# duj12/ASR-2Pass

Hardware: AMD Instinct MI355X
Metric: audio-sec/sec (xRT) Paraformer-large offline, 30s utts (higher is better)
Workload: dtype f32 (operands staged as 2 fp16 planes = 22-23 significant bits, 3 products per block on the FP16 matrix cores, fp32 accumulate; error vs fp64 = the fp32 MFMA chain's)

## Files before the change

### asr-2pass_amd/csrc/gemm_p3.hip

```cpp
#include "kernels.h"
#include "launch_common.h"
#include "split_common.h"

#include <algorithm>
#include <atomic>

namespace pfhip {
namespace {

using f32x16 = __attribute__((ext_vector_type(16))) float;

constexpr int kPM = 128, kPN = 128, kPK = 16;
constexpr int kPRowB = 32;
constexpr int kPPlane = 128 * kPRowB;
constexpr int kPStage = 4 * kPPlane;
constexpr int kPRing = 4;
constexpr int kPCs = kPN + 4;
constexpr int kPLds = kPM * kPCs * 4 + kPM * 8;
static_assert(kPRing * kPStage <= kPLds, "the ring must fit");

__device__ __forceinline__ size_t image_off(int kstep, int row, int piece, int rows) {
  return ((size_t)kstep * rows + row) * kPRowB + (size_t)((piece ^ ((row >> 3) & 1)) << 4);
}

// ... 203 lines not shown
#define PFHIP_S3(kt) PFHIP_STEP(ga_, gb_, fa, fb, 3, 0, kclamp((kt) + 7))
  int kt = 0;
  for (; kt + 3 < nk; kt += 4) { PFHIP_S0(kt) PFHIP_S1(kt) PFHIP_S2(kt) PFHIP_S3(kt) }
  if (kt < nk) PFHIP_S0(kt)
  if (kt + 1 < nk) PFHIP_S1(kt)
  if (kt + 2 < nk) PFHIP_S2(kt)
#undef PFHIP_S0
#undef PFHIP_S1
#undef PFHIP_S2
#undef PFHIP_S3
#undef PFHIP_STEP
#undef PFHIP_D1
#undef PFHIP_M
#undef PFHIP_RA
#undef PFHIP_RB
#undef PFHIP_DMA
#undef PFHIP_DMA1
#undef PFHIP_SB
  PFHIP_STAMP
  asm volatile("s_waitcnt vmcnt(0)" ::: "memory");
  __syncthreads();
  PFHIP_STAMP
#ifndef PFHIP_P3_EPI
#define PFHIP_P3_EPI 0
#endif
  if (PFHIP_P3_EPI == 2) {
    if (M < 0) C[tid] = acc00[0] + acc01[1] + acc10[2] + acc11[3];
    return;
  }
#ifndef PFHIP_P3_STAMPS
  const bool do_store = PFHIP_P3_EPI != 1 || M < 0;
#endif

  float* const Cs = reinterpret_cast<float*>(lds);
  {
    float* cw = Cs + (wr * 64 + 4 * h) * kPCs + wc * 64 + r;
#pragma unroll
    for (int e = 0; e < 16; ++e) {
      const int ro = ((e & 3) + 8 * (e >> 2)) * kPCs;
      cw[ro] = acc00[e];
      cw[ro + 32] = acc01[e];
      cw[ro + 32 * kPCs] = acc10[e];
      cw[ro + 32 * kPCs + 32] = acc11[e];
    }
  }
  float2* const s_mr = reinterpret_cast<float2*>(lds + kPM * kPCs * 4);
  if (LN && tid < kPM) s_mr[tid] = ln_mr;
  __syncthreads();
  PFHIP_STAMP
#ifdef PFHIP_P3_STAMPS
  const bool do_store = !stamp_wg;
#define PFHIP_P3_STAMP_END if (stamping) { asm volatile("s_waitcnt vmcnt(0)" ::: "memory"); *dbg_at(n_stamp) = __builtin_amdgcn_s_memtime(); *dbg_at(n_stamp + 1) = __builtin_amdgcn_s_memrealtime(); }
#else
#define PFHIP_P3_STAMP_END
#endif

  if (kv_tile) {
    row_planes_tile<LN, kPM, kPThreads>(Cs, s_mr, m0, n0, M, N, inv_scale, bias, ln_colsum, Ph, Pl, rows_p, split_col, tid, do_store);
  } else if (OUT & 1) {
    const int c4 = e_c4, rsub = e_rsub, gcol = e_gcol;
    float4 cv[16];
    float2 mrv[16];
#pragma unroll
    for (int pass = 0; pass < 16; ++pass) {
      const int row = pass * 8 + rsub;
      cv[pass] = *reinterpret_cast<const float4*>(Cs + row * kPCs + 4 * c4);
      mrv[pass] = LN ? s_mr[row] : make_float2(0.f, 1.f);
    }
#ifdef PFHIP_P3_STAMPS
    { float keep = cv[15].x + mrv[15].x; asm volatile("" : "+v"(keep)); }
    PFHIP_STAMP
#endif
#pragma unroll
    for (int pass = 0; pass < 16; ++pass) {
      const int row = pass * 8 + rsub, grow = m0 + row;
      float4 v = cv[pass];
      v.x *= inv_scale; v.y *= inv_scale; v.z *= inv_scale; v.w *= inv_scale;
      if (LN) {
        const float2 mr = mrv[pass];
        v.x = mr.y * (v.x - mr.x * e_cs.x); v.y = mr.y * (v.y - mr.x * e_cs.y); v.z = mr.y * (v.z - mr.x * e_cs.z); v.w = mr.y * (v.w - mr.x * e_cs.w);
      }
      v.x += e_bv.x + e_r1[pass].x; v.y += e_bv.y + e_r1[pass].y; v.z += e_bv.z + e_r1[pass].z; v.w += e_bv.w + e_r1[pass].w;
      if (relu) { v.x = fmaxf(v.x, 0.f); v.y = fmaxf(v.y, 0.f); v.z = fmaxf(v.z, 0.f); v.w = fmaxf(v.w, 0.f); }
      if (do_store && grow < M && e_cols) *reinterpret_cast<float4*>(C + (size_t)grow * ldc + gcol) = v;
      if (OUT & 2) *reinterpret_cast<float4*>(Cs + row * kPCs + 4 * c4) = v;
      if (stats_out) tile_row_stats(v, grow, M, tn, tiles_n, c4, stats_out);
    }
#ifdef PFHIP_P3_STAMPS
    PFHIP_STAMP
#endif
    if (OUT & 2) __syncthreads();
  }
  if (OUT & 2) {
    const int row = tid & 127, grow = m0 + row;
    const float2 mr = (LN && OUT == 2) ? s_mr[row] : make_float2(0.f, 1.f);
#pragma unroll
    for (int jj = 0; jj < 4; ++jj) {
      const int j = (tid >> 7) + 2 * jj;
      float v[16];
#pragma unroll
      for (int c = 0; c < 4; ++c) {
        const float4 t = *reinterpret_cast<const float4*>(Cs + row * kPCs + 16 * j + 4 * c);
        v[4 * c] = t.x; v[4 * c + 1] = t.y; v[4 * c + 2] = t.z; v[4 * c + 3] = t.w;
      }
      if (OUT == 2) {
        const int gc = n0 + 16 * j;
#pragma unroll
        for (int c = 0; c < 4; ++c) {
          const float4 b4 = bias ? *reinterpret_cast<const float4*>(bias + gc + 4 * c) : make_float4(0.f, 0.f, 0.f, 0.f);
          const float4 s4 = LN ? *reinterpret_cast<const float4*>(ln_colsum + gc + 4 * c) : make_float4(0.f, 0.f, 0.f, 0.f);
          const float bb[4] = {b4.x, b4.y, b4.z, b4.w}, ss[4] = {s4.x, s4.y, s4.z, s4.w};
#pragma unroll
          for (int e = 0; e < 4; ++e) {
            float x = v[4 * c + e] * inv_scale;
            if (LN) x = mr.y * (x - mr.x * ss[e]);
            x += bb[e];
            if (relu) x = fmaxf(x, 0.f);
            v[4 * c + e] = x;
          }
        }
      }
      const int ksp = (n0 >> 4) + j;
#pragma unroll
      for (int pc = 0; pc < 2; ++pc) {
        const float w8[8] = {v[8 * pc], v[8 * pc + 1], v[8 * pc + 2], v[8 * pc + 3], v[8 * pc + 4], v[8 * pc + 5], v[8 * pc + 6], v[8 * pc + 7]};
        uint4 hh, ll;
        split8(w8, hh, ll);
        const size_t off = image_off(ksp, grow, pc, rows_p);
        if (do_store) {
          *reinterpret_cast<uint4*>(Ph + off) = hh;
          *reinterpret_cast<uint4*>(Pl + off) = ll;
        } else if (hh.x == 0x12345678u && ll.y == 0x9abcdef0u) {
          Ph[0] = 1;
        }
      }
    }
  }
  PFHIP_P3_STAMP_END
}
#undef PFHIP_P3_STAMP_END
#undef PFHIP_STAMP

constexpr int kQM = 256;
constexpr int kQThreads = 512;
constexpr int kQAPlane = kQM * kPRowB;
constexpr int kQWOff = 2 * kQAPlane;
constexpr int kQStage = kQWOff + 2 * kPPlane;
constexpr int kQLds = kPRing * kQStage;
static_assert(kPM * kPCs * 4 + kQM * 8 <= kQLds, "half of the C tile and the row statistics must fit the ring");
template <bool LN, int OUT>
__global__ __launch_bounds__(kQThreads, 2) void gemm_p3_256_kernel(
    const unsigned char* __restrict__ Ah, const unsigned char* __restrict__ Al, int rows_a, const unsigned char* __restrict__ Wh,
    const unsigned char* __restrict__ Wl, int rows_w, float* C, int ldc, unsigned char* __restrict__ Ph, unsigned char* __restrict__ Pl,
    int rows_p, const float* __restrict__ bias, const float* R1, int ldr1, int M, int N, int K, int tiles_n, int n_tiles, int gw, int relu,
    const float* __restrict__ ln_stats, int ln_tiles, float ln_eps, const float* __restrict__ ln_colsum, float* __restrict__ stats_out,
    float inv_scale, int* range_flag, int split_col) {
  extern __shared__ __attribute__((aligned(16))) unsigned char lds[];

  int tm, tn;
  tile_of_block(blockIdx.x, n_tiles, tiles_n, gw, tm, tn);
  const int m0 = tm * kQM, n0 = tn * kPN;
  const int tid = threadIdx.x, lane = tid & 63, wave = tid >> 6;
  const int wr = wave >> 1, wc = wave & 1;
  const int r = lane & 31, h = lane >> 5;

  const size_t ka = (size_t)rows_a * kPRowB, kw = (size_t)rows_w * kPRowB;
  const int arow = min(m0 + 32 * wave, rows_a - 32);
// ... 40 lines not shown
    PFHIP_QDMA1(gww + (size_t)(kdma) * kw, (wst) * kQStage + lds_w) PFHIP_SB;                                         \
    PFHIP_M(acc01, FA[0][0], FB[0][1])                                                                                \
    PFHIP_M(acc10, FA[0][1], FB[0][0])                                                                                \
    PFHIP_M(acc11, FA[0][1], FB[0][1])                                                                                \
    asm volatile("s_waitcnt vmcnt(6) lgkmcnt(0)\n\ts_barrier" ::: "memory");                                          \
    PFHIP_SB;                                                                                                         \
  }

  const int nk = K / kPK;
  auto kclamp = [&](int t) { return t < nk ? t : nk - 1; };
  PFHIP_QDMA(0, 0)
  PFHIP_QDMA(1, kclamp(1))
  PFHIP_QDMA(2, kclamp(2))
  PFHIP_QDMA(3, kclamp(3))
  asm volatile("s_waitcnt vmcnt(6)\n\ts_barrier" ::: "memory");
  PFHIP_RA(fa, 0, 0, 0) PFHIP_RA(fa, 0, 0, 1) PFHIP_RA(fa, 0, 1, 0) PFHIP_RA(fa, 0, 1, 1)
  PFHIP_RB(fb, 0, 0, 0) PFHIP_RB(fb, 0, 0, 1) PFHIP_RB(fb, 0, 1, 0) PFHIP_RB(fb, 0, 1, 1)
  asm volatile("s_waitcnt lgkmcnt(0)\n\ts_barrier" ::: "memory");
#define PFHIP_S0(kt) PFHIP_STEP(fa, fb, ga_, gb_, 0, 1, kclamp((kt) + 4))
#define PFHIP_S1(kt) PFHIP_STEP(ga_, gb_, fa, fb, 1, 2, kclamp((kt) + 5))
#define PFHIP_S2(kt) PFHIP_STEP(fa, fb, ga_, gb_, 2, 3, kclamp((kt) + 6))
#define PFHIP_S3(kt) PFHIP_STEP(ga_, gb_, fa, fb, 3, 0, kclamp((kt) + 7))
  int kt = 0;
  for (; kt + 3 < nk; kt += 4) { PFHIP_S0(kt) PFHIP_S1(kt) PFHIP_S2(kt) PFHIP_S3(kt) }
  if (kt < nk) PFHIP_S0(kt)
  if (kt + 1 < nk) PFHIP_S1(kt)
  if (kt + 2 < nk) PFHIP_S2(kt)
#undef PFHIP_S0
#undef PFHIP_S1
#undef PFHIP_S2
#undef PFHIP_S3
#undef PFHIP_STEP
#undef PFHIP_M
#undef PFHIP_RA
#undef PFHIP_RB
#undef PFHIP_QDMA
#undef PFHIP_QDMA1
#undef PFHIP_SB
  asm volatile("s_waitcnt vmcnt(0)" ::: "memory");
  __syncthreads();

  float* const Cs = reinterpret_cast<float*>(lds);
  float2* const s_mr = reinterpret_cast<float2*>(lds + kPM * kPCs * 4);
  if (LN && tid < kQM) s_mr[tid] = ln_mr;
#pragma unroll 1
  for (int hf = 0; hf < 2; ++hf) {
    if ((wr >> 1) == hf) {
      float* cw = Cs + ((wr & 1) * 64 + 4 * h) * kPCs + wc * 64 + r;
#pragma unroll
      for (int e = 0; e < 16; ++e) {
        const int ro = ((e & 3) + 8 * (e >> 2)) * kPCs;
        cw[ro] = acc00[e];
        cw[ro + 32] = acc01[e];
        cw[ro + 32 * kPCs] = acc10[e];
        cw[ro + 32 * kPCs + 32] = acc11[e];
      }
    }
    __syncthreads();
    const int mh = m0 + 128 * hf;
    if (OUT & 1) {
      const int c4 = tid & 31, rsub = tid >> 5;
      const int gcol = n0 + 4 * c4;
      float4 bv = make_float4(0.f, 0.f, 0.f, 0.f), cs4 = bv;
      if (bias && gcol + 3 < N) bv = *reinterpret_cast<const float4*>(bias + gcol);
      if (LN && gcol + 3 < N) cs4 = *reinterpret_cast<const float4*>(ln_colsum + gcol);
      float4 r1v[8];
#pragma unroll
      for (int pass = 0; pass < 8; ++pass) {
        const int grow = mh + pass * 16 + rsub;
        r1v[pass] = (R1 && grow < M && gcol + 3 < N) ? *reinterpret_cast<const float4*>(R1 + (size_t)grow * ldr1 + gcol)
                                                     : make_float4(0.f, 0.f, 0.f, 0.f);
      }
#pragma unroll
      for (int pass = 0; pass < 8; ++pass) {
        const int row = pass * 16 + rsub, grow = mh + row;
        float4 v = *reinterpret_cast<const float4*>(Cs + row * kPCs + 4 * c4);
        v.x *= inv_scale; v.y *= inv_scale; v.z *= inv_scale; v.w *= inv_scale;
        if (LN) {
          const float2 mr = s_mr[128 * hf + row];
          v.x = mr.y * (v.x - mr.x * cs4.x); v.y = mr.y * (v.y - mr.x * cs4.y); v.z = mr.y * (v.z - mr.x * cs4.z); v.w = mr.y * (v.w - mr.x * cs4.w);
        }
        v.x += bv.x + r1v[pass].x; v.y += bv.y + r1v[pass].y; v.z += bv.z + r1v[pass].z; v.w += bv.w + r1v[pass].w;
        if (relu) { v.x = fmaxf(v.x, 0.f); v.y = fmaxf(v.y, 0.f); v.z = fmaxf(v.z, 0.f); v.w = fmaxf(v.w, 0.f); }
        if (grow < M && gcol + 3 < N) *reinterpret_cast<float4*>(C + (size_t)grow * ldc + gcol) = v;
        if (OUT & 2) *reinterpret_cast<float4*>(Cs + row * kPCs + 4 * c4) = v;
        if (stats_out) tile_row_stats(v, grow, M, tn, tiles_n, c4, stats_out);
      }
      if (OUT & 2) __syncthreads();
    }
    if (OUT & 2) {
      const int row = tid & 127, grow = mh + row;
      const float2 mr = (LN && OUT == 2) ? s_mr[128 * hf + row] : make_float2(0.f, 1.f);
#pragma unroll
      for (int jj = 0; jj < 2; ++jj) {
        const int j = (tid >> 7) + 4 * jj;
        float v[16];
#pragma unroll
        for (int c = 0; c < 4; ++c) {
          const float4 t = *reinterpret_cast<const float4*>(Cs + row * kPCs + 16 * j + 4 * c);
          v[4 * c] = t.x; v[4 * c + 1] = t.y; v[4 * c + 2] = t.z; v[4 * c + 3] = t.w;
        }
        if (OUT == 2) {
          const int gc = n0 + 16 * j;
#pragma unroll
          for (int c = 0; c < 4; ++c) {
            const float4 b4 = bias ? *reinterpret_cast<const float4*>(bias + gc + 4 * c) : make_float4(0.f, 0.f, 0.f, 0.f);
            const float4 s4 = LN ? *reinterpret_cast<const float4*>(ln_colsum + gc + 4 * c) : make_float4(0.f, 0.f, 0.f, 0.f);
            const float bb[4] = {b4.x, b4.y, b4.z, b4.w}, ss[4] = {s4.x, s4.y, s4.z, s4.w};
#pragma unroll
            for (int e = 0; e < 4; ++e) {
              float x = v[4 * c + e] * inv_scale;
              if (LN) x = mr.y * (x - mr.x * ss[e]);
              x += bb[e];
              if (relu) x = fmaxf(x, 0.f);
              v[4 * c + e] = x;
            }
          }
        }
        const int ksp = (n0 >> 4) + j;
        if (grow < rows_p) {
#pragma unroll
          for (int pc = 0; pc < 2; ++pc) {
            const float w8[8] = {v[8 * pc], v[8 * pc + 1], v[8 * pc + 2], v[8 * pc + 3], v[8 * pc + 4], v[8 * pc + 5], v[8 * pc + 6], v[8 * pc + 7]};
            uint4 hh, ll;
            split8(w8, hh, ll);
            const size_t off = image_off(ksp, grow, pc, rows_p);
            *reinterpret_cast<uint4*>(Ph + off) = hh;
            *reinterpret_cast<uint4*>(Pl + off) = ll;
          }
        }
      }
    }
    __syncthreads();
  }
}

template <bool LN, int OUT>
__device__ __forceinline__ void epilogue_rows64(const int tid, float* const Cs, const float2* const s_mr, const int m0, const int n0, const int tn,
                                                const int tiles_n, float* C, int ldc, unsigned char* __restrict__ Ph, unsigned char* __restrict__ Pl,
                                                int rows_p, const float* __restrict__ bias, const float* R1, int ldr1, int M, int N, int relu,
                                                const float* __restrict__ ln_colsum, float* __restrict__ stats_out, float inv_scale, int split_col) {
  if ((OUT & 4) && n0 >= split_col) {
    row_planes_tile<LN, 64, kPThreads>(Cs, s_mr, m0, n0, M, N, inv_scale, bias, ln_colsum, Ph, Pl, rows_p, split_col, tid, true);
  } else if (OUT & 1) {
    const int c4 = tid & 31, rsub = tid >> 5;
    const int gcol = n0 + 4 * c4;
    float4 bv = make_float4(0.f, 0.f, 0.f, 0.f), cs4 = bv;
    if (bias && gcol + 3 < N) bv = *reinterpret_cast<const float4*>(bias + gcol);
    if (LN && gcol + 3 < N) cs4 = *reinterpret_cast<const float4*>(ln_colsum + gcol);
    float4 r1v[8];
#pragma unroll
    for (int pass = 0; pass < 8; ++pass) {
      const int grow = m0 + pass * 8 + rsub;
      r1v[pass] = (R1 && grow < M && gcol + 3 < N) ? *reinterpret_cast<const float4*>(R1 + (size_t)grow * ldr1 + gcol)
                                                   : make_float4(0.f, 0.f, 0.f, 0.f);
    }
#pragma unroll
    for (int pass = 0; pass < 8; ++pass) {
      const int row = pass * 8 + rsub, grow = m0 + row;
      float4 v = *reinterpret_cast<const float4*>(Cs + row * kPCs + 4 * c4);
      v.x *= inv_scale; v.y *= inv_scale; v.z *= inv_scale; v.w *= inv_scale;
      if (LN) {
        const float2 mr = s_mr[row];
        v.x = mr.y * (v.x - mr.x * cs4.x); v.y = mr.y * (v.y - mr.x * cs4.y); v.z = mr.y * (v.z - mr.x * cs4.z); v.w = mr.y * (v.w - mr.x * cs4.w);
      }
      v.x += bv.x + r1v[pass].x; v.y += bv.y + r1v[pass].y; v.z += bv.z + r1v[pass].z; v.w += bv.w + r1v[pass].w;
      if (relu) { v.x = fmaxf(v.x, 0.f); v.y = fmaxf(v.y, 0.f); v.z = fmaxf(v.z, 0.f); v.w = fmaxf(v.w, 0.f); }
      if (grow < M && gcol + 3 < N) *reinterpret_cast<float4*>(C + (size_t)grow * ldc + gcol) = v;
      if (OUT & 2) *reinterpret_cast<float4*>(Cs + row * kPCs + 4 * c4) = v;
      if (stats_out) tile_row_stats(v, grow, M, tn, tiles_n, c4, stats_out);
    }
    if (OUT & 2) __syncthreads();
  }
  if (OUT & 2) {
    const int row = tid & 63, grow = m0 + row;
    const float2 mr = (LN && OUT == 2) ? s_mr[row] : make_float2(0.f, 1.f);
#pragma unroll
    for (int jj = 0; jj < 2; ++jj) {
      const int j = (tid >> 6) + 4 * jj;
      float v[16];
#pragma unroll
      for (int c = 0; c < 4; ++c) {
        const float4 t = *reinterpret_cast<const float4*>(Cs + row * kPCs + 16 * j + 4 * c);
        v[4 * c] = t.x; v[4 * c + 1] = t.y; v[4 * c + 2] = t.z; v[4 * c + 3] = t.w;
      }
      if (OUT == 2) {
        const int gc = n0 + 16 * j;
#pragma unroll
        for (int c = 0; c < 4; ++c) {
          const float4 b4 = bias ? *reinterpret_cast<const float4*>(bias + gc + 4 * c) : make_float4(0.f, 0.f, 0.f, 0.f);
          const float4 s4 = LN ? *reinterpret_cast<const float4*>(ln_colsum + gc + 4 * c) : make_float4(0.f, 0.f, 0.f, 0.f);
          const float bb[4] = {b4.x, b4.y, b4.z, b4.w}, ss[4] = {s4.x, s4.y, s4.z, s4.w};
#pragma unroll
          for (int e = 0; e < 4; ++e) {
            float x = v[4 * c + e] * inv_scale;
            if (LN) x = mr.y * (x - mr.x * ss[e]);
            x += bb[e];
            if (relu) x = fmaxf(x, 0.f);
            v[4 * c + e] = x;
          }
        }
      }
      const int ksp = (n0 >> 4) + j;
#pragma unroll
      for (int pc = 0; pc < 2; ++pc) {
        const float w8[8] = {v[8 * pc], v[8 * pc + 1], v[8 * pc + 2], v[8 * pc + 3], v[8 * pc + 4], v[8 * pc + 5], v[8 * pc + 6], v[8 * pc + 7]};
        uint4 hh, ll;
        split8(w8, hh, ll);
        const size_t off = image_off(ksp, grow, pc, rows_p);
        *reinterpret_cast<uint4*>(Ph + off) = hh;
        *reinterpret_cast<uint4*>(Pl + off) = ll;
      }
    }
  }
}

constexpr int kHM = 64;
constexpr int kHAPlane = kHM * kPRowB;
constexpr int kHWOff = 2 * kHAPlane;
constexpr int kHStage = kHWOff + 2 * kPPlane;
constexpr int kHLds = kPRing * kHStage;
static_assert(kHM * kPCs * 4 + kHM * 8 <= kHLds, "the C tile must fit the ring");
template <bool LN, int OUT>
__global__ __launch_bounds__(kPThreads, 3) void gemm_p3_64_kernel(
    const unsigned char* __restrict__ Ah, const unsigned char* __restrict__ Al, int rows_a, const unsigned char* __restrict__ Wh,
    const unsigned char* __restrict__ Wl, int rows_w, float* C, int ldc, unsigned char* __restrict__ Ph, unsigned char* __restrict__ Pl,
    int rows_p, const float* __restrict__ bias, const float* R1, int ldr1, int M, int N, int K, int tiles_n, int n_tiles, int gw, int relu,
    const float* __restrict__ ln_stats, int ln_tiles, float ln_eps, const float* __restrict__ ln_colsum, float* __restrict__ stats_out,
    float inv_scale, int* range_flag, int split_col) {
  extern __shared__ __attribute__((aligned(16))) unsigned char lds[];

  int tm, tn;
  tile_of_block(blockIdx.x, n_tiles, tiles_n, gw, tm, tn);
  const int m0 = tm * kHM, n0 = tn * kPN;
  const int tid = threadIdx.x, lane = tid & 63, wave = tid >> 6;
  const int wr = wave >> 1, wc = wave & 1;
  const int r = lane & 31, h = lane >> 5;

  const size_t ka = (size_t)rows_a * kPRowB, kw = (size_t)rows_w * kPRowB;
  const unsigned char* const ga = ((wave >> 1) ? Al : Ah) + ((size_t)(m0 + 32 * (wave & 1))) * kPRowB + lane * 16;
  const unsigned char* const gwh = Wh + ((size_t)(n0 + 32 * wave)) * kPRowB + lane * 16;
  const unsigned char* const gwl = Wl + ((size_t)(n0 + 32 * wave)) * kPRowB + lane * 16;
  const int lds_a = (wave >> 1) * kHAPlane + (wave & 1) * 1024, lds_w = kHWOff + wave * 1024;
#define PFHIP_DMA1(src, off)                                                                                           \
  __builtin_amdgcn_global_load_lds((const __attribute__((address_space(1))) void*)(src),                              \
                                   (__attribute__((address_space(3))) void*)(lds + (off)), 16, 0, 0);
#define PFHIP_DMA(stage, ks)                                                                                          \
  PFHIP_DMA1(ga + (size_t)(ks) * ka, (stage) * kHStage + lds_a) PFHIP_DMA1(gwh + (size_t)(ks) * kw, (stage) * kHStage + lds_w)     \
  PFHIP_DMA1(gwl + (size_t)(ks) * kw, (stage) * kHStage + lds_w + kPPlane)

  const int ra = wr * 32 + r, rb = wc * 64 + r;
// ... 476 lines not shown

size_t plane_image_bytes(int rows, int K) { return (size_t)((rows + 127) / 128 * 128) * (size_t)K * 2; }

void launch_split_planes(const float* X, int ld, int rows_valid, int rows, int K, float scale, void* hi, void* lo, hipStream_t s) {
  if (rows <= 0 || K <= 0) return;
  const size_t n = (size_t)rows * (K / 8);
  hipLaunchKernelGGL(split_planes_kernel, dim3((unsigned)((n + 255) / 256)), dim3(256), 0, s, X, ld, rows_valid, rows, K, scale,
                     static_cast<unsigned char*>(hi), static_cast<unsigned char*>(lo));
}

namespace {
std::atomic<long> g_wide_launches{0};
int cu_count() {
  static std::atomic<int> cus[64];
  int dev = 0;
  (void)hipGetDevice(&dev);
  int n = cus[dev & 63].load(std::memory_order_relaxed);
  if (n <= 0) {
    if (hipDeviceGetAttribute(&n, hipDeviceAttributeMultiprocessorCount, dev) != hipSuccess || n <= 0) n = 256;
    cus[dev & 63].store(n, std::memory_order_relaxed);
  }
  return n;
}
int half_tiles_limit() {
  static const int lim = env_int("PFHIP_P3_HALF_TILES", 400);
  return lim;
}
char tile256_knob() {
  static const char c = [] { const char* e = getenv("PFHIP_P3_TILE256"); return e ? e[0] : '\0'; }();
  return c;
}
}
long gemm_p3_wide_launches() { return g_wide_launches.load(std::memory_order_relaxed); }
bool gemm_p3_wide_serves(bool c, bool planes, bool r1, bool ln, bool stats_out, int row_planes_from, int N, int K) {
  return ln && c != planes && !r1 && !stats_out && row_planes_from <= 0 && N > 0 && N % kWN == 0 && K >= kPK && K % kPK == 0;
}

#ifndef PFHIP_P3_LDS_PAD
#define PFHIP_P3_LDS_PAD 0
#endif
void launch_gemm_p3(const PlaneGemmOp& o, hipStream_t s, int tile_rows, int tile_cols) {
  const int M = o.M, N = o.N, K = o.K, rows_a = o.rows_a, row_planes_from = o.row_planes_from, rl = o.relu ? 1 : 0;
  float* const C = o.C;
  if (M <= 0 || N <= 0) return;
  constexpr int kGroupWidth = 4;
  const float inv = 1.0f / o.w_scale;
  const unsigned char *ah = static_cast<const unsigned char*>(o.Ah), *al = static_cast<const unsigned char*>(o.Al);
  const unsigned char *wh = static_cast<const unsigned char*>(o.Wh), *wl = static_cast<const unsigned char*>(o.Wl);
  unsigned char *ph = static_cast<unsigned char*>(o.Ph), *pl = static_cast<unsigned char*>(o.Pl);
  {
    const bool serves = gemm_p3_wide_serves(C != nullptr, o.Ph != nullptr, o.R1 != nullptr, o.ln_stats != nullptr, o.stats_out != nullptr, row_planes_from, N, K);
    const int nw = ((M + kWM - 1) / kWM) * (N / kWN), cus = cu_count(), rounds = (nw + cus - 1) / cus;
    const bool w_env = env_on("PFHIP_P3_WIDE");
    const int half_lim = half_tiles_limit();
    const bool by_rule = tile_cols == 0 && tile_rows == 0 && w_env && serves && o.ln_tiles == 4 && K >= 256 && rows_a >= kWM && nw > cus &&
                         ((M + kPM - 1) / kPM) * ((N + kPN - 1) / kPN) > half_lim && 100 * nw >= 85 * cus * rounds;
    if (serves && (tile_cols == kWN || by_rule)) {
      const int grid = (nw + rounds - 1) / rounds;
      const int tn = N / kWN, g = std::max(1, std::min(kGroupWidth, tn));
      g_wide_launches.fetch_add(1, std::memory_order_relaxed);
      if (C)
        launch_with_lds<gemm_p3_256x256_kernel<true, 1>, kWThreads>(grid, kWLds, s, ah, al, rows_a, wh, wl, o.rows_w, C, o.ldc, nullptr, nullptr, o.rows_p, o.bias,
                                                                    M, N, K, tn, nw, g, rl, o.ln_stats, o.ln_tiles, 1e-12f, o.ln_colsum, inv, launch_ctx().range_flag);
      else
        launch_with_lds<gemm_p3_256x256_kernel<true, 2>, kWThreads>(grid, kWLds, s, ah, al, rows_a, wh, wl, o.rows_w, nullptr, 0, ph, pl, o.rows_p, o.bias, M, N, K,
                                                                    tn, nw, g, rl, o.ln_stats, o.ln_tiles, 1e-12f, o.ln_colsum, inv, launch_ctx().range_flag);
      return;
    }
  }
  const int tiles_n = (N + kPN - 1) / kPN;
  const int half_env = half_tiles_limit();
  const bool half = tile_rows == kHM || (tile_rows != kPM && tile_rows != kQM && ((M + kPM - 1) / kPM) * tiles_n <= half_env);
  const bool q_env = tile256_knob() != '0';
  const int nq = ((M + kQM - 1) / kQM) * tiles_n;
  const bool q_all = tile256_knob() == '2';
  const bool quad = row_planes_from <= 0 && (tile_rows == kQM || (tile_rows == 0 && q_env && !half && rows_a >= kQM && (K >= 1024 || q_all) &&
                                         100 * nq >= 85 * 256 * ((nq + 255) / 256)));
  const int r3_env = env_int("PFHIP_P3_R3", -1);
  const bool ring3 = !quad && !half && (r3_env == 1 || (r3_env != 0 && ((M + kPM - 1) / kPM) * tiles_n > 1536));
  const int tmr = quad ? kQM : (half ? kHM : kPM);
  const int n_tiles = ((M + tmr - 1) / tmr) * tiles_n;
  static const int gw_env = env_int("PFHIP_P3_GW", 0);
  const int gw = std::max(1, std::min(gw_env > 0 ? gw_env : kGroupWidth, tiles_n));
  const int out = (C ? 1 : 0) | (ph ? 2 : 0);
#define PFHIP_P3_GO(THREADS, LDS, ...)                                                                                                        \
  launch_with_lds<__VA_ARGS__, THREADS>(n_tiles, LDS, s, ah, al, rows_a, wh, wl, o.rows_w, C, o.ldc, ph, pl, o.rows_p, o.bias, o.R1, o.ldr1, M, N, K, \
                                        tiles_n, n_tiles, gw, rl, o.ln_stats, o.ln_tiles, 1e-12f, o.ln_colsum, o.stats_out, inv,              \
                                        launch_ctx().range_flag, row_planes_from)
#define PFHIP_P3(LNF, OUTM)                                                                              \
  {                                                                                                      \
    if (quad) PFHIP_P3_GO(kQThreads, kQLds, gemm_p3_256_kernel<LNF, OUTM>);                              \
    else if (half) PFHIP_P3_GO(kPThreads, kHLds, gemm_p3_64_kernel<LNF, OUTM>);                          \
    else if (ring3) PFHIP_P3_GO(kPThreads, kP3Lds, gemm_p3_128r3_kernel<LNF, OUTM>);                     \
    else PFHIP_P3_GO(kPThreads, kPLds + PFHIP_P3_LDS_PAD, gemm_p3_128_kernel<LNF, OUTM>);                \
  }
  if (row_planes_from > 0) {
    if (half && o.ln_stats) PFHIP_P3_GO(kPThreads, kHLds, gemm_p3_64_kernel<true, 5>);
    else if (half) PFHIP_P3_GO(kPThreads, kHLds, gemm_p3_64_kernel<false, 5>);
    else if (o.ln_stats) PFHIP_P3_GO(kPThreads, kPLds, gemm_p3_128_kernel<true, 5>);
    else PFHIP_P3_GO(kPThreads, kPLds, gemm_p3_128_kernel<false, 5>);
    return;
  }
  if (o.ln_stats) {
    if (out == 1) PFHIP_P3(true, 1) else if (out == 2) PFHIP_P3(true, 2) else PFHIP_P3(true, 3)
  } else {
    if (out == 1) PFHIP_P3(false, 1) else if (out == 2) PFHIP_P3(false, 2) else PFHIP_P3(false, 3)
  }
#undef PFHIP_P3
#undef PFHIP_P3_GO
}

}
```

### asr-2pass_amd/csrc/kernels.h

```cpp
#pragma once
#include <hip/hip_runtime.h>
#include <stdint.h>

namespace pfhip {

constexpr int kTileM = 128;
constexpr int kTileN = 128;
constexpr int kTileK = 32;
constexpr int kHeadDim = 128;
constexpr int kHeadDimSmall = 80;
inline bool head_dim_supported(int hd) { return hd == kHeadDim || hd == kHeadDimSmall; }
constexpr int kMelW = 32;

struct FbankTables {
  const float* window;
  const double* tw512;
  const int* mel_off;
  const int* mel_size;
  const float* mel_w;
  const float* cmvn_mean;
  const float* cmvn_istd;
};
void launch_fbank_lfr_cmvn(const float* pcm, const int64_t* sample_off, const int* frame_off,
                           const int* nframes, const int* row_off, int B, int total_frames,
                           FbankTables tb, float* feats, hipStream_t s);
void launch_fbank_lfr_cmvn(const int16_t* pcm, const int64_t* sample_off, const int* frame_off,
                           const int* nframes, const int* row_off, int B, int total_frames,
                           FbankTables tb, float* feats, hipStream_t s);

void launch_fbank_frames(const float* pcm, const int64_t* sample_off, const int* frame_off, const int* nframes,
                         int total_frames, FbankTables tb, float* fb_out, hipStream_t s);
void launch_fbank_frames(const int16_t* pcm, const int64_t* sample_off, const int* frame_off, const int* nframes,
                         int total_frames, FbankTables tb, float* fb_out, hipStream_t s);
void launch_fbank_frames_batch(const float* pcm, const int64_t* sample_off, const int* frame_off, const int* nframes, int B,
                               int total_frames, FbankTables tb, float* fb_out, hipStream_t s);
void launch_fbank_frames_batch(const int16_t* pcm, const int64_t* sample_off, const int* frame_off, const int* nframes, int B,
                               int total_frames, FbankTables tb, float* fb_out, hipStream_t s);

void launch_embed(const float* feats, int D, float* x0, int ldx, const int* row_pos, int M,
                  const float* inv_timescale, float scale, hipStream_t s);

struct LaunchCtx {
  bool exact = false;
  int* range_flag = nullptr;
};
LaunchCtx& launch_ctx();
constexpr float kLnRstdMin = 1.0f / 2048.0f, kLnRstdMax = 256.0f;
constexpr float kLnOffsetMax = 4.0f;
__host__ __device__ inline bool ln_row_out_of_domain(float mean, float rstd) {
  const float off = mean * rstd;
  return !(rstd > kLnRstdMin && rstd < kLnRstdMax) || !(off * off <= kLnOffsetMax * kLnOffsetMax);
}

struct GemmOp {
  const float* A = nullptr; int lda = 0;
  const float* W = nullptr; int ldw = 0;
  float* C = nullptr; int ldc = 0;
  int M = 0, N = 0, K = 0;
  const float* bias = nullptr;
  const float* R1 = nullptr; int ldr1 = 0;
  const float* R2 = nullptr; int ldr2 = 0;
  bool relu = false;
  float w_scale = 1.0f;
  const float* ln_stats = nullptr; int ln_tiles = 0; const float* ln_colsum = nullptr;
  float* stats_out = nullptr;
};
enum class GemmKernel { BySize, Tiled128, Streaming, Tiled64, Bf16_256, Bf16_128, Bf16_64, F16_256, F16_128, F16_64, SplitBySize };
enum class SplitTile { Rows256, Rows128, Rows64 };
enum class SplitForm { ByContext, F16x3, Bf16x6 };
void launch_gemm(const GemmOp& op, GemmKernel kernel, bool guard, hipStream_t s);
float best_w_scale(float max_abs);
void launch_gemm_f32_bf16x6(const GemmOp& op, SplitTile tile, int gw, hipStream_t s);
void launch_gemm_f32_f16x3(const GemmOp& op, SplitTile tile, int gw, hipStream_t s);
size_t plane_image_bytes(int rows, int K);
void launch_split_planes(const float* X, int ld, int rows_valid, int rows, int K, float scale, void* hi, void* lo, hipStream_t s);
struct PlaneGemmOp {
  const void* Ah = nullptr; const void* Al = nullptr; int rows_a = 0;
  const void* Wh = nullptr; const void* Wl = nullptr; int rows_w = 0;
  float w_scale = 1.0f;
  float* C = nullptr; int ldc = 0;
  void* Ph = nullptr; void* Pl = nullptr; int rows_p = 0;
  int row_planes_from = 0;
  int M = 0, N = 0, K = 0;
  const float* bias = nullptr;
  const float* R1 = nullptr; int ldr1 = 0;
  bool relu = false;
  const float* ln_stats = nullptr; int ln_tiles = 0; const float* ln_colsum = nullptr;
  float* stats_out = nullptr;
};
void launch_gemm_p3(const PlaneGemmOp& op, hipStream_t s,
                    int tile_rows = 0,
                    int tile_cols = 0);
bool gemm_p3_wide_serves(bool c, bool planes, bool r1, bool ln, bool stats_out, int row_planes_from, int N, int K);
long gemm_p3_wide_launches();
void launch_split_rows(const float* X, int ld, int rows, int cols, void* hi, void* lo, int ldp, hipStream_t s);
bool gemm_x6_ln_ok(int M);
bool gemm_f16_planes_form();

void launch_layernorm(const float* x, int ldx, float* y, int ldy, const float* g, const float* b,
                      int M, int D, int Dout, float eps, hipStream_t s);

void launch_fsmn(const float* v, int ldv, const float* w, const float* res, int ldres, float* out,
                 int ldo, const int* off, const int* len, int B, int max_len, int C, hipStream_t s);
void launch_fsmn_shift(const float* v, int ldv, const float* w, const float* res, int ldres, float* out,
                       int ldo, const int* off, const int* len, int B, int max_len, int C, int shift, hipStream_t s);

struct AttnOp {
  const float* Q = nullptr; int ldq = 0;
  const float* K = nullptr; int ldk = 0;
  const float* V = nullptr; int ldv = 0;
  float* O = nullptr; int ldo = 0;
  const int* q_off = nullptr; const int* q_len = nullptr;
  const int* kv_off = nullptr; const int* kv_len = nullptr;
  int B = 0, H = 0, max_q_len = 0;
  float scale = 1.0f;
  int head_dim = kHeadDim;
  const int* q_kv_limit = nullptr;
  const float* fsmn_w = nullptr; float* mem = nullptr; int ldmem = 0; bool mem_accumulate = false;
  void* planes_hi = nullptr; void* planes_lo = nullptr; int plane_rows = 0;
  const void* kv_hi = nullptr; const void* kv_lo = nullptr; int ldkv = 0, v_col = 0;
};
void launch_attention(const AttnOp& op, hipStream_t s);
void launch_attention_x6(const AttnOp& op, hipStream_t s);
void launch_attention_x3(const AttnOp& op, hipStream_t s);
void launch_attention_p3(const AttnOp& op, hipStream_t s);
void launch_attention_h80(const AttnOp& op, hipStream_t s);
void launch_attention_dk(const AttnOp& op, hipStream_t s);
void launch_attention_fsmn(const AttnOp& op, hipStream_t s);
bool attention_planes_ok(int max_len, int head_dim = kHeadDim);
bool attention_fsmn_is_fused(int max_len, int head_dim = kHeadDim);

constexpr int kBlstmScratchFloats = 2 * 4 * 32 * 512 + 8;
constexpr int kBlstmFlagWord = 2 * 4 * 32 * 512 + 2;
hipError_t launch_blstm(const float* gx, const float* whh, float* y, float* hx, const int* off, const int* len, int B, int Lmax,
                        hipStream_t s);
hipError_t launch_blstm_stepwise(const float* gx, const float* whh, float* y, float* hx, float* cst, const int* off, const int* len, int B,
                                 int Lmax, hipStream_t s);
void launch_alpha2(const float* y, int ldy, const float* w, float b, float smooth, float noise, float* a2, int rows, int D,
                   hipStream_t s);
void launch_us_cif(const float* a2, const int* off, const int* len, const int* token_num, int B, int max_len, float threshold,
                   float* us_alphas, float* us_peaks, hipStream_t s);

void launch_im2col3(const float* h, int ldh, float* col, int ldc, const int* row_pos,
                    const int* row_len, int M, int D, hipStream_t s);
void launch_alpha(const float* o, int ldo, const float* w, const float* b, float smooth,
                  float noise, float* alphas, int M, int D, hipStream_t s);
void launch_cif(const float* hidden, int ldh, const float* alphas, const int* row_off,
                const int* len, int B, int D, float threshold, float tail, float* stage,
                int* n_fires, int* token_num, hipStream_t s, int* fire_frame = nullptr);
void launch_compact(const float* stage, float* emb, const int* tok_row_src, int ML, int D,
                    hipStream_t s);

void launch_gather_rows(const int32_t* ids, const float* table, int D, float* out, int R, hipStream_t s);
void launch_lstm_cell(const float* G, float* c, float* h, const int32_t* lens, int t, float* sel, int H, int D,
                      hipStream_t s);

void launch_logsoftmax_argmax(const float* logits, int ldl, int ML, int V, float* logp, int32_t* ids,
                              hipStream_t s, int* range_flag = nullptr);
size_t ctc_head_workspace_bytes(int M, int V);
bool launch_ctc_head(const float* X, int ldx, const float* W, int ldw, const float* bias, float w_scale, int M, int V, int K, int32_t* ids,
                     float* logp_best, float* lse, void* workspace, size_t workspace_bytes, hipStream_t s, int* range_flag = nullptr);
void launch_svs_prompt_rows(const float* E, int D, const int* prompt, const int* row_off, const int* len, int B, float* feats, int ld,
                            hipStream_t s);
void launch_gather_best(const float* logp, int ld, const int32_t* ids, int M, float* best, hipStream_t s);
void launch_row_lse(const float* logits, int ld, int M, int V, float* lse, hipStream_t s);
int ctc_collapse_chunk();
bool launch_ctc_collapse(const int32_t* frame_ids, const float* frame_logp, const int* row_off, const int* len, int B, int blank,
                         int max_tokens, int32_t* ids, int32_t* tok_frame, float* tok_logp, int32_t* token_num, hipStream_t s);
bool launch_ctc_emissions(const float* X, int ldx, const float* W, int ldw, const float* bias, const float* lse, const int* row_off,
                          const int* len, const int* lab_off, const int* n_lab, const int32_t* labels, const long long* e_off, int B, int K,
                          int V, int blank, float* E, hipStream_t s);
size_t ctc_align_workspace_bytes(size_t e_floats);
int ctc_align_max_tokens();
bool launch_ctc_align(const float* E, const long long* e_off, size_t e_floats, const int* len, const int* n_lab, const int32_t* labels,
                      const int* lab_off, int B, int max_tokens, int32_t* tok_begin, int32_t* tok_end, float* tok_logp, float* score,
                      void* workspace, size_t workspace_bytes, hipStream_t s);
constexpr int kTopkMax = 8;
bool launch_logsoftmax_topk(const float* logits, int ldl, int ML, int V, int k, float* logp, int32_t* ids, int32_t* topk_ids,
                            float* topk_logp, hipStream_t s, int* range_flag = nullptr);

void launch_stream_lfr(const float* fb, int T, int n_rows, const float* mean, const float* istd, float scale,
                       const float* inv_ts, int pos0, float* out, int ldo, hipStream_t s);
void launch_rows_copy(float* dst, int ldd, const float* src, int lds_, int nrows, int ncols, hipStream_t s);
struct RowsCopyOp { float* dst; const float* src; int ldd, lds, nrows, ncols; };
struct StreamLfrOp { const float* fb; float* out; int T, n_rows, pos0, pad_; };
void launch_rows_copy_batch(const RowsCopyOp* ops, int n_ops, int max_rows, hipStream_t s);
// ... 69 lines not shown
```

### asr-2pass_amd/csrc/ops_abi.cpp

```cpp
#include "../../include/pfhip_ops.h"

#include "kernels.h"

#include <vector>

namespace {
inline hipStream_t S(void* s) { return static_cast<hipStream_t>(s); }
inline int done() { return (int)hipGetLastError(); }
template <class Seg, class Launch>
int with_device_segs(const std::vector<Seg>& host, hipStream_t s, Launch launch) {
  Seg* d = nullptr;
  hipError_t e = hipMalloc(reinterpret_cast<void**>(&d), host.size() * sizeof(Seg));
  if (e != hipSuccess) return (int)e;
  e = hipMemcpy(d, host.data(), host.size() * sizeof(Seg), hipMemcpyHostToDevice);
  if (e == hipSuccess) {
    launch(d);
    e = hipGetLastError();
    const hipError_t e2 = hipStreamSynchronize(s);
    if (e == hipSuccess) e = e2;
  }
  (void)hipFree(d);
  return (int)e;
}
constexpr int kKindBySize = 0;
// ... 55 lines not shown
  const pfhip::LnGemmRoute r = pfhip::fused_ln_gemm_route(M, N, K, has_ln != 0);
  const int v[6] = {(int)r.kernel, r.ln, r.cw, r.mr, r.waves, r.k_blocks};
  for (int i = 0; i < 6; ++i) out[i] = v[i];
  return 0;
}
int pfhip_dev_fused_gemv_1trip_bench(const float* X, int ldx, const float* W, int ldw, size_t w_stride_floats, int n_copies, float* C, int ldc,
                                     const float* bias, const float* ln_colsum, const float* R1, int ldr1, int M, int N, int K, int relu,
                                     int n_launch, void* stream) {
  for (int i = 0; i < n_launch; ++i)
    if (!pfhip::launch_fused_gemv_1trip(X, ldx, W + (size_t)(i % n_copies) * w_stride_floats, ldw, C, ldc, bias, ln_colsum, 1e-12f, R1, ldr1,
                                        nullptr, 0, nullptr, M, N, K, relu != 0, S(stream)))
      return (int)hipErrorInvalidValue;
  return done();
}
int pfhip_op_window_attention(const float* Q, int ldq, const float* K, int ldk, const float* V, int ldv, float* O, int ldo, int Lq, int Lk,
                              int H, float scale, void* stream) {
  if (!pfhip::launch_window_attention(Q, ldq, K, ldk, V, ldv, O, ldo, Lq, Lk, H, scale, S(stream))) return (int)hipErrorInvalidValue;
  return done();
}
int pfhip_op_window_attention_hd(const float* Q, int ldq, const float* K, int ldk, const float* V, int ldv, float* O, int ldo, int Lq, int Lk,
                                 int H, float scale, int head_dim, void* stream) {
  if (head_dim != 128 && head_dim != 80) return (int)hipErrorInvalidValue;
  if (!pfhip::launch_window_attention(Q, ldq, K, ldk, V, ldv, O, ldo, Lq, Lk, H, scale, S(stream), head_dim)) return (int)hipErrorInvalidValue;
  return done();
}
int pfhip_op_window_attention_segments(const float* Q, int ldq, const float* K, int ldk, const float* V, int ldv, float* O, int ldo,
                                       const int* q_off, const int* q_len, const int* kv_off, const int* kv_len, int B, int H, int max_q_len,
                                       int max_kv_len, float scale, const float* fsmn_w, float* mem, int ldmem, int head_dim, void* stream) {
  if ((head_dim != 128 && head_dim != 80) || B < 1 || H < 1 || max_q_len < 1 || max_q_len > 32 || max_kv_len < 1 || max_kv_len > 32 ||
      !Q || !K || !V || !O || !q_off || !q_len || !kv_off || !kv_len)
    return (int)hipErrorInvalidValue;
  const long long w = (long long)H * head_dim;
  if ((ldq | ldk | ldv | ldo) % 4 || ldq < w || ldk < w || ldv < w || ldo < w || (fsmn_w && (!mem || ldmem < w || ldmem % 4)))
    return (int)hipErrorInvalidValue;
  if (!pfhip::launch_window_attention_segments(Q, ldq, K, ldk, V, ldv, O, ldo, q_off, q_len, kv_off, kv_len, B, H, max_q_len, max_kv_len, scale,
                                               S(stream), fsmn_w, mem, ldmem, head_dim))
    return (int)hipErrorInvalidValue;
  return done();
}
int pfhip_op_fused_att_out(const float* Q, int ldq, const float* K, int ldk, const float* V, int ldv, int Lq, int Lk, int H, float scale,
                           const float* W, int ldw, float* C, int ldc, const float* bias, const float* R1, int ldr1, const float* fsmn_v,
                           int ldfv, const float* fsmn_w, int N, void* stream) {
  if (!pfhip::launch_fused_att_out(Q, ldq, K, ldk, V, ldv, Lq, Lk, H, scale, W, ldw, C, ldc, bias, R1, ldr1, fsmn_v, ldfv, fsmn_w, N, S(stream)))
    return (int)hipErrorInvalidValue;
  return done();
}
int pfhip_op_gemm_f32_scaled(const float* A, int lda, const float* W, int ldw, float* C, int ldc, const float* bias, const float* R1,
                             int ldr1, const float* R2, int ldr2, int M, int N, int K, int relu, int guard, int kind, float w_scale,
                             void* stream) {
  pfhip::GemmKernel kernel;
  if (K % pfhip::kTileK || !kernel_of_kind(kind, &kernel) || !(w_scale > 0.f)) return (int)hipErrorInvalidValue;
  pfhip::launch_gemm({.A = A, .lda = lda, .W = W, .ldw = ldw, .C = C, .ldc = ldc, .M = M, .N = N, .K = K, .bias = bias, .R1 = R1, .ldr1 = ldr1,
                      .R2 = R2, .ldr2 = ldr2, .relu = relu != 0, .w_scale = w_scale},
                     kernel, guard != 0, S(stream));
  return (int)hipGetLastError();
}
float pfhip_op_best_w_scale(float max_abs) { return pfhip::best_w_scale(max_abs); }
int pfhip_op_set_launch_ctx(int* range_flag, int exact) {
  pfhip::launch_ctx().range_flag = range_flag;
  pfhip::launch_ctx().exact = exact != 0;
  return 0;
}
int pfhip_op_gemm_f32_ln(const float* A, int lda, const float* W, int ldw, float* C, int ldc, const float* bias, const float* R1, int ldr1,
                         const float* R2, int ldr2, int M, int N, int K, int relu, const float* ln_stats, int ln_tiles,
                         const float* ln_colsum, float* stats_out, float w_scale, void* stream) {
  if (M <= 0 || N <= 0 || K < pfhip::kTileK || K % pfhip::kTileK || !A || !W || !C || lda < K || ldw < K || ldc < N || (R1 && ldr1 < N) ||
      (R2 && ldr2 < N) || (lda | ldw | ldc | ldr1 | ldr2) % 4 || !(w_scale > 0.f) || (ln_stats && (!ln_colsum || ln_tiles <= 0 || N % 4)) || (!ln_stats && ln_colsum) ||
      (stats_out && N % 128))
    return (int)hipErrorInvalidValue;
  pfhip::launch_gemm({.A = A, .lda = lda, .W = W, .ldw = ldw, .C = C, .ldc = ldc, .M = M, .N = N, .K = K, .bias = bias, .R1 = R1, .ldr1 = ldr1,
                      .R2 = R2, .ldr2 = ldr2, .relu = relu != 0, .w_scale = w_scale, .ln_stats = ln_stats, .ln_tiles = ln_tiles,
                      .ln_colsum = ln_colsum, .stats_out = stats_out},
                     pfhip::GemmKernel::SplitBySize, false, S(stream));
  return (int)hipGetLastError();
}

size_t pfhip_op_plane_image_bytes(int rows, int K) { return pfhip::plane_image_bytes(rows, K); }
int pfhip_op_split_planes(const float* X, int ld, int rows_valid, int rows, int K, float scale, void* hi, void* lo, void* stream) {
  if (K < 16 || K % 16 || rows <= 0 || rows % 128 || rows_valid < 0 || rows_valid > rows || !hi || !lo || (rows_valid > 0 && (!X || ld < K)))
    return (int)hipErrorInvalidValue;
  pfhip::launch_split_planes(X, ld, rows_valid, rows, K, scale, hi, lo, S(stream));
  return (int)hipGetLastError();
}
int pfhip_op_gemm_p3(const void* Ah, const void* Al, int rows_a, const void* Wh, const void* Wl, int rows_w, float w_scale, float* C, int ldc,
                     void* Ph, void* Pl, int rows_p, const float* bias, const float* R1, int ldr1, int M, int N, int K, int relu,
                     const float* ln_stats, int ln_tiles, const float* ln_colsum, float* stats_out, int tile_rows, void* stream) {
  const int mp = (M + 127) / 128 * 128;
  if (M <= 0 || N <= 0 || K < 16 || K % 16 || N % 128 || rows_a % 128 || rows_w % 128 || rows_a < mp || rows_w < N || !Ah || !Al || !Wh ||
      !Wl || (!C && !Ph) || (Ph && (!Pl || rows_p % 128 || rows_p < mp)) || (C && ldc < N) || (R1 && ldr1 < N) || !(w_scale > 0.f) ||
      (ln_stats && (!ln_colsum || ln_tiles <= 0)) || (stats_out && !C)  ||
      (tile_rows != 0 && tile_rows != 64 && tile_rows != 128 && tile_rows != 256))
    return (int)hipErrorInvalidValue;
  pfhip::launch_gemm_p3({.Ah = Ah, .Al = Al, .rows_a = rows_a, .Wh = Wh, .Wl = Wl, .rows_w = rows_w, .w_scale = w_scale, .C = C, .ldc = ldc,
                         .Ph = Ph, .Pl = Pl, .rows_p = rows_p, .M = M, .N = N, .K = K, .bias = bias, .R1 = R1, .ldr1 = ldr1,
                         .relu = relu != 0, .ln_stats = ln_stats, .ln_tiles = ln_tiles, .ln_colsum = ln_colsum, .stats_out = stats_out},
                        S(stream), tile_rows);
  return (int)hipGetLastError();
}
int pfhip_op_gemm_p3_cols(const void* Ah, const void* Al, int rows_a, const void* Wh, const void* Wl, int rows_w, float w_scale, float* C, int ldc,
                          void* Ph, void* Pl, int rows_p, const float* bias, const float* R1, int ldr1, int M, int N, int K, int relu,
                          const float* ln_stats, int ln_tiles, const float* ln_colsum, float* stats_out, int tile_rows, int tile_cols, void* stream) {
  if (tile_cols == 0)
    return pfhip_op_gemm_p3(Ah, Al, rows_a, Wh, Wl, rows_w, w_scale, C, ldc, Ph, Pl, rows_p, bias, R1, ldr1, M, N, K, relu, ln_stats, ln_tiles, ln_colsum,
                            stats_out, tile_rows, stream);
  const int mp = (M + 127) / 128 * 128;
  if (tile_cols != 256 || tile_rows != 0 || M <= 0 || N <= 0 || K < 16 || K % 16 || N % 256 || rows_a % 128 || rows_w % 128 || rows_a < mp ||
      rows_w < N || !Ah || !Al || !Wh || !Wl || (Ph && (!Pl || rows_p % 128 || rows_p < mp)) || (C && ldc < N) || !(w_scale > 0.f) ||
      (ln_stats && (!ln_colsum || ln_tiles <= 0)) ||
      !pfhip::gemm_p3_wide_serves(C != nullptr, Ph != nullptr, R1 != nullptr, ln_stats != nullptr, stats_out != nullptr, 0, N, K))
    return (int)hipErrorInvalidValue;
  pfhip::launch_gemm_p3({.Ah = Ah, .Al = Al, .rows_a = rows_a, .Wh = Wh, .Wl = Wl, .rows_w = rows_w, .w_scale = w_scale, .C = C, .ldc = ldc,
                         .Ph = Ph, .Pl = Pl, .rows_p = rows_p, .M = M, .N = N, .K = K, .bias = bias, .relu = relu != 0,
                         .ln_stats = ln_stats, .ln_tiles = ln_tiles, .ln_colsum = ln_colsum},
                        S(stream), 0, 256);
  return (int)hipGetLastError();
}
long pfhip_op_gemm_p3_wide_launches(void) { return pfhip::gemm_p3_wide_launches(); }

int pfhip_op_layernorm(const float* x, int ldx, float* y, int ldy, const float* g, const float* b, int M, int D,
                       int Dout, float eps, void* stream) {
  if (D % 4 || Dout % 4 || Dout > 2048 || D > Dout) return (int)hipErrorInvalidValue;
  pfhip::launch_layernorm(x, ldx, y, ldy, g, b, M, D, Dout, eps, S(stream));
  return done();
}
int pfhip_op_fsmn(const float* v, int ldv, const float* w, const float* res, int ldres, float* out, int ldo,
                  const int* off, const int* len, int B, int max_len, int C, void* stream) {
  if (C % 4) return (int)hipErrorInvalidValue;
  pfhip::launch_fsmn(v, ldv, w, res, ldres, out, ldo, off, len, B, max_len, C, S(stream));
  return done();
}
int pfhip_op_fsmn_shift(const float* v, int ldv, const float* w, const float* res, int ldres, float* out, int ldo,
                        const int* off, const int* len, int B, int max_len, int C, int shift, void* stream) {
  if ((shift != 0 && shift != 5) || C <= 0 || C % 4 || !v || !w || !out || !off || !len || (ldv | ldo) % 4 || ldv < C || ldo < C ||
      (res && (ldres % 4 || ldres < C)))
    return (int)hipErrorInvalidValue;
  pfhip::launch_fsmn_shift(v, ldv, w, res, ldres, out, ldo, off, len, B, max_len, C, shift, S(stream));
  return done();
}
int pfhip_op_attention_limit(const float* Q, int ldq, const float* K, int ldk, const float* V, int ldv, float* O, int ldo,
                             const int* q_off, const int* q_len, const int* kv_off, const int* kv_len, int B, int H,
                             int max_q_len, float scale, int head_dim, const int* q_kv_limit, void* stream) {
  if ((head_dim != 32 && head_dim != 80 && head_dim != 128) || H < 1 || !Q || !K || !V || !O || !q_off || !q_len || !kv_off || !kv_len ||
      !q_kv_limit)
    return (int)hipErrorInvalidValue;
  const long long w = (long long)H * head_dim;
  if ((ldq | ldk | ldv | ldo) % 4 || ldq < w || ldk < w || ldv < w || ldo < w) return (int)hipErrorInvalidValue;
  pfhip::launch_attention({.Q = Q, .ldq = ldq, .K = K, .ldk = ldk, .V = V, .ldv = ldv, .O = O, .ldo = ldo, .q_off = q_off, .q_len = q_len, .kv_off = kv_off, .kv_len = kv_len, .B = B, .H = H,
                           .max_q_len = max_q_len, .scale = scale, .head_dim = head_dim, .q_kv_limit = q_kv_limit},
                          S(stream));
  return done();
}
int pfhip_op_attention(const float* Q, int ldq, const float* K, int ldk, const float* V, int ldv, float* O, int ldo,
                       const int* q_off, const int* q_len, const int* kv_off, const int* kv_len, int B, int H,
                       int max_q_len, float scale, void* stream) {
  return pfhip_op_attention_hd(Q, ldq, K, ldk, V, ldv, O, ldo, q_off, q_len, kv_off, kv_len, B, H, max_q_len, scale, pfhip::kHeadDim, stream);
}
int pfhip_op_attention_hd(const float* Q, int ldq, const float* K, int ldk, const float* V, int ldv, float* O, int ldo,
                          const int* q_off, const int* q_len, const int* kv_off, const int* kv_len, int B, int H,
                          int max_q_len, float scale, int head_dim, void* stream) {
  if (head_dim != 32 && head_dim != 80 && head_dim != 128) return (int)hipErrorInvalidValue;
  pfhip::launch_attention({.Q = Q, .ldq = ldq, .K = K, .ldk = ldk, .V = V, .ldv = ldv, .O = O, .ldo = ldo, .q_off = q_off, .q_len = q_len, .kv_off = kv_off, .kv_len = kv_len, .B = B, .H = H,
                           .max_q_len = max_q_len, .scale = scale, .head_dim = head_dim},
                          S(stream));
  return done();
}
int pfhip_op_attention_dk(const float* Q, int ldq, const float* K, int ldk, const float* V, int ldv, float* O, int ldo,
                          const int* q_off, const int* q_len, const int* kv_off, const int* kv_len, int B, int H,
                          int max_q_len, float scale, int d_k, const int* q_kv_limit, void* stream) {
  if (d_k < 1 || d_k > 64 || H < 1 || !Q || !K || !V || !O || !q_off || !q_len || !kv_off || !kv_len) return (int)hipErrorInvalidValue;
  const long long w = (long long)H * d_k;
  if (ldq < w || ldk < w || ldv < w || ldo < w) return (int)hipErrorInvalidValue;
  pfhip::launch_attention_dk({.Q = Q, .ldq = ldq, .K = K, .ldk = ldk, .V = V, .ldv = ldv, .O = O, .ldo = ldo, .q_off = q_off, .q_len = q_len, .kv_off = kv_off, .kv_len = kv_len, .B = B, .H = H,
                              .max_q_len = max_q_len, .scale = scale, .head_dim = d_k, .q_kv_limit = q_kv_limit},
                             S(stream));
  return done();
}
int pfhip_op_attention_fsmn(const float* Q, int ldq, const float* K, int ldk, const float* V, int ldv, float* O, int ldo, const int* off,
                            const int* len, int B, int H, int max_len, float scale, const float* fsmn_w, float* mem, int ldmem,
                            int mem_accumulate, int head_dim, void* stream) {
  if ((head_dim != 80 && head_dim != 128) || !fsmn_w || !mem || !O || H <= 0 || ldmem < H * head_dim) return (int)hipErrorInvalidValue;
  pfhip::launch_attention_fsmn({.Q = Q, .ldq = ldq, .K = K, .ldk = ldk, .V = V, .ldv = ldv, .O = O, .ldo = ldo, .q_off = off, .q_len = len, .kv_off = off, .kv_len = len, .B = B, .H = H, .max_q_len = max_len,
                                .scale = scale, .head_dim = head_dim, .fsmn_w = fsmn_w, .mem = mem, .ldmem = ldmem,
                                .mem_accumulate = mem_accumulate != 0},
                               S(stream));
  return done();
}
int pfhip_op_attention_fsmn_is_fused(int max_len, int head_dim) { return pfhip::attention_fsmn_is_fused(max_len, head_dim) ? 1 : 0; }
int pfhip_op_attention_planes(const float* Q, int ldq, const float* K, int ldk, const float* V, int ldv, void* planes_hi, void* planes_lo,
                              int plane_rows, const int* q_off, const int* q_len, const int* kv_off, const int* kv_len, int B, int H,
                              int max_q_len, int total_q_rows, float scale, void* stream) {
  if (!planes_hi || !planes_lo || plane_rows % 128 || total_q_rows > plane_rows || B <= 0 || H <= 0) return (int)hipErrorInvalidValue;
  pfhip::launch_attention_x3({.Q = Q, .ldq = ldq, .K = K, .ldk = ldk, .V = V, .ldv = ldv, .q_off = q_off, .q_len = q_len, .kv_off = kv_off,
                              .kv_len = kv_len, .B = B, .H = H, .max_q_len = max_q_len, .scale = scale, .planes_hi = planes_hi,
                              .planes_lo = planes_lo, .plane_rows = plane_rows},
                             S(stream));
  return done();
}
int pfhip_op_split_rows(const float* X, int ld, int rows, int cols, void* hi, void* lo, int ldp, void* stream) {
  if (!X || !hi || !lo || rows <= 0 || cols <= 0 || cols % 8 || ld < cols || ldp < cols || ldp % 8) return (int)hipErrorInvalidValue;
  pfhip::launch_split_rows(X, ld, rows, cols, hi, lo, ldp, S(stream));
  return (int)hipGetLastError();
}
int pfhip_op_gemm_p3_qkv(const void* Ah, const void* Al, int rows_a, const void* Wh, const void* Wl, int rows_w, float w_scale, float* C, int ldc,
                         void* kv_hi, void* kv_lo, int ldkv, int q_cols, const float* bias, int M, int N, int K, const float* ln_stats,
                         int ln_tiles, const float* ln_colsum, int tile_rows, void* stream) {
  const int mp = (M + 127) / 128 * 128;
  if (M <= 0 || N <= 0 || K < 16 || K % 16 || N % 128 || rows_a % 128 || rows_w % 128 || rows_a < mp || rows_w < N || !Ah || !Al || !Wh ||
      !Wl || !C || !kv_hi || !kv_lo || q_cols <= 0 || q_cols % 128 || q_cols >= N || ldc < q_cols || ldkv < N - q_cols || ldkv % 8 ||
      !(w_scale > 0.f) || (ln_stats && (!ln_colsum || ln_tiles <= 0)) || (tile_rows != 0 && tile_rows != 64 && tile_rows != 128))
    return (int)hipErrorInvalidValue;
  pfhip::launch_gemm_p3({.Ah = Ah, .Al = Al, .rows_a = rows_a, .Wh = Wh, .Wl = Wl, .rows_w = rows_w, .w_scale = w_scale, .C = C, .ldc = ldc,
// ... 196 lines not shown
```

### asr-2pass_amd/csrc/pfhip.cpp

```cpp
#include "../../include/pfhip.h"

#include <hip/hip_runtime.h>

#include <algorithm>
#include <chrono>
#include <cmath>
#include <cstdio>
#include <cstdlib>
#include <cstring>
#include <fstream>
#include <map>
#include <mutex>
#include <optional>
#include <sstream>
#include <string>
#include <unordered_map>
#include <vector>

#include "internal.h"
#include "launch_common.h"
#include "json_min.h"

namespace pfhip_impl {
std::atomic<uint64_t>& buf_epoch() {
// ... 896 lines not shown
    const pfhip_status rs = read_range_flag(m, s, false);
    if (rs) return rs;
  }
  HIP_TRY(hipStreamSynchronize(s));
  HIP_TRY(hipGetLastError());
  m->range_hit = m->h_flag.p ? *m->h_flag.i() : 0;
  const SvsHost h = svs_host(m);
  for (int b = 0; b < B; ++b) {
    m->token_num[b] = h.num[b];
    m->maxL = std::max(m->maxL, h.num[b]);
  }
  return PFHIP_OK;
}

pfhip_status forward_cif(pfhip_model* m, hipStream_t s) {
  const ModelWeights& w = *m->weights;
  const Config& c = w.cfg;
  const int d = c.d_model, B = m->B, M = m->M;
  float* col = m->qkv.f();
  float* po = m->ctx.f();
  {
    Scope sc(m, s, K_OTHER, 0, 16.0 * M * d);
    pfhip::launch_im2col3(m->enc.f(), d, col, 3 * d, m->m_row_pos, m->m_row_len, M, d, s);
  }
  gemm(m, s, col, 3 * d, w.pred.conv, d, 3 * d, 3 * d, po, d, c.pred_residual ? m->enc.f() : nullptr, d, nullptr, 0, M, true);
  {
    Scope sc(m, s, K_OTHER, 2.0 * M * d, 4.0 * M * d);
    pfhip::launch_alpha(po, d, w.pred.out_w, w.pred.out_b, c.smooth_factor, c.noise_threshold, m->alphas.f(), M, d, s);
  }
  float* stage = m->hbuf.f();
  int* fire = m->want_fires ? m->counts.i() + 2 * B : nullptr;
  {
    Scope sc(m, s, K_CIF, 2.0 * M * d, 4.0 * M * d);
    pfhip::launch_cif(m->enc.f(), d, m->alphas.f(), m->m_row_off, m->m_len, B, d, c.cif_threshold, c.tail_threshold,
                      stage, m->counts.i(), m->counts.i() + B, s, fire);
  }
  m->have_fires = fire != nullptr;
  const int* h_counts = m->h_counts.i();
  HIP_TRY(hipMemcpyAsync(m->h_counts.p, m->counts.p, ((size_t)2 * B + (fire ? (size_t)M + B : 0)) * 4, hipMemcpyDeviceToHost, s));
  HIP_TRY(hipStreamSynchronize(s));
  int ML = 0;
  for (int b = 0; b < B; ++b) {
    m->n_fires[b] = h_counts[b];
    m->token_num[b] = h_counts[B + b];
    m->tok_off[b] = ML;
    ML += m->n_fires[b];
    m->maxL = std::max(m->maxL, m->n_fires[b]);
  }
  m->ML = ML;
  if (ML == 0) HIP_TRY(hipGetLastError());
  return PFHIP_OK;
}

pfhip_status forward_decoder(pfhip_model* m, hipStream_t s, const ForwardPaths& paths) {
  const ModelWeights& w = *m->weights;
  const Config& c = w.cfg;
  const int d = c.d_model, B = m->B, M = m->M, ML = m->ML;
  const int Mp = round_up(M, pfhip::kTileM);
  if (c.contextual) {
    bool have = m->fw_hwkv != nullptr && (int)m->fw_hw_len.size() == B;
    for (int b = 0; have && b < B; ++b) have = m->fw_hw_len[b] > 0;
    if (!have) return fail(PFHIP_ERR_ARG, "contextual model needs hotword embeddings (pfhip_set_hotwords / hw_emb)");
  }
  const int MLp = round_up(ML, pfhip::kTileM);

  {
    const size_t n = 4 * (size_t)B + ML;
    HIP_TRY(m->dmeta.ensure(n * 4));
    if (m->h_meta.cap / 2 + n * 4 > m->h_meta.cap) return fail(PFHIP_ERR_CAPACITY, "internal: metadata staging too small");
    int* hm = reinterpret_cast<int*>(static_cast<char*>(m->h_meta.p) + m->h_meta.cap / 2);
    int* dm = m->dmeta.i();
    std::memcpy(hm, m->tok_off.data(), 4 * B); m->m_tok_off = dm;
    std::memcpy(hm + B, m->n_fires.data(), 4 * B); m->m_tok_len = dm + B;
    for (int b = 0; b < B; ++b) { hm[2 * B + b] = c.contextual ? m->fw_hw_off[b] : 0; hm[3 * B + b] = c.contextual ? m->fw_hw_len[b] : 0; }
    m->m_hw_off = dm + 2 * B; m->m_hw_len = dm + 3 * B;
    m->m_src_row = dm + 4 * B;
    for (int b = 0; b < B; ++b)
      for (int n2 = 0; n2 < m->n_fires[b]; ++n2) hm[4 * B + m->tok_off[b] + n2] = m->row_off[b] + b + n2;
    HIP_TRY(hipMemcpyAsync(dm, hm, n * 4, hipMemcpyHostToDevice, s));
  }
  HIP_TRY(m->emb.ensure((size_t)MLp * d * 4));
  HIP_TRY(m->xd.ensure((size_t)MLp * d * 4));
  HIP_TRY(m->yd.ensure((size_t)MLp * d * 4));
  HIP_TRY(m->hd.ensure((size_t)MLp * c.dec_ffn * 4));
  HIP_TRY(m->hd2.ensure((size_t)MLp * c.dec_ffn * 4));
  HIP_TRY(m->td.ensure((size_t)MLp * d * 4));
  HIP_TRY(m->t2.ensure((size_t)MLp * d * 4));
  HIP_TRY(m->qd.ensure((size_t)MLp * d * 4));
  HIP_TRY(m->ctxd.ensure((size_t)MLp * d * 4));
  HIP_TRY(m->logits.ensure((size_t)MLp * w.vocab_pad * 4));
  HIP_TRY(m->ids.ensure((size_t)MLp * 4));
  if (m->nbest_k) { HIP_TRY(m->nb_ids.ensure((size_t)MLp * m->nbest_k * 4)); HIP_TRY(m->nb_logp.ensure((size_t)MLp * m->nbest_k * 4)); }
  {
    Scope sc(m, s, K_OTHER, 0, 8.0 * ML * d);
    pfhip::launch_compact(m->hbuf.f(), m->emb.f(), m->m_src_row, ML, d, s);
    HIP_TRY(hipMemcpyAsync(m->xd.p, m->emb.p, (size_t)ML * d * 4, hipMemcpyDeviceToDevice, s));
  }

  float* xd = m->xd.f();
  float* kvbuf = m->qkv.f();
  static const bool side_on = pfhip::env_is1("PFHIP_DEC_SIDE");
  const bool side_kv = side_on && c.dec_layers > 0 && M >= 4096 && m->side_stream;
  if (side_kv) {
    HIP_TRY(m->kvside.ensure((size_t)c.dec_layers * Mp * 2 * d * 4));
    HIP_TRY(hipEventRecord(m->ev_enc_ready, s));
    HIP_TRY(hipStreamWaitEvent(m->side_stream, m->ev_enc_ready, 0));
    for (int i = 0; i < c.dec_layers; ++i) {
      gemm(m, m->side_stream, m->enc.f(), d, w.dec[(size_t)i].kv, 2 * d, d, d, m->kvside.f() + (size_t)i * Mp * 2 * d, 2 * d,
           nullptr, 0, nullptr, 0, M, false);
      HIP_TRY(hipEventRecord(m->ev_kv[(size_t)i], m->side_stream));
    }
  }
  double cross_pairs = 0;
  for (int b = 0; b < B; ++b) cross_pairs += (double)m->n_fires[b] * m->T[b];
  const int hdd = d / c.dec_n_head;
  const float att_scale_d = 1.0f / sqrtf((float)hdd);
  const bool fuse_dec = w.dec_folded && pfhip::gemm_x6_ln_ok(ML) && !pfhip::launch_ctx().exact;
  const int ftiles = c.dec_ffn / pfhip::kTileN;
  if (fuse_dec) {
    HIP_TRY(m->lnstats.ensure((size_t)std::max(Mp, MLp) * 4 * 2 * 4));
    HIP_TRY(m->lnstats2.ensure((size_t)MLp * ftiles * 2 * 4));
  }
  auto x6ln = [&](const Linear& W, pfhip::GemmOp op) {
    const int N = op.N, K = op.K;
    Scope sc(m, s, K_GEMM, 2.0 * ML * (double)N * K, 4.0 * ((double)ML * K + (double)N * K + (double)ML * N));
    op.lda = op.ldw = K; op.W = W.w; op.bias = W.b; op.w_scale = W.scale; op.ldc = N; op.M = ML; op.ldr1 = d;
    pfhip::launch_gemm(op, pfhip::GemmKernel::SplitBySize, false, s);
  };
  bool xd_has_stats = false;
  static const int dec_planes_min_rows = pfhip::env_int("PFHIP_DEC_PLANES_MIN_ROWS", 3500);
  const bool dec_planes = paths.planes && fuse_dec && w.dec_planes && ML >= dec_planes_min_rows && pfhip::attention_planes_ok(m->maxL, hdd) &&
                          pfhip::gemm_f16_planes_form();
  Img encP{nullptr, nullptr}, xdP{nullptr, nullptr}, hdP{nullptr, nullptr}, ctxdP{nullptr, nullptr};
  bool xd_has_planes = false;
  if (dec_planes) {
    ++m->dec_plane_forwards;
    const size_t pe = pfhip::plane_image_bytes(Mp, d), pdd = pfhip::plane_image_bytes(MLp, d), pff = pfhip::plane_image_bytes(MLp, c.dec_ffn);
    HIP_TRY(m->encP.ensure(2 * pe));
    HIP_TRY(m->xdP.ensure(2 * pdd));
    HIP_TRY(m->ctxP.ensure(2 * pdd));
    HIP_TRY(m->hP.ensure(2 * pff));
    encP = img_of(m->encP, pe); xdP = img_of(m->xdP, pdd); ctxdP = img_of(m->ctxP, pdd); hdP = img_of(m->hP, pff);
    Scope sc(m, s, K_OTHER, 0, 8.0 * M * d);
    pfhip::launch_split_planes(m->enc.f(), d, M, Mp, d, 1.0f, encP.hi, encP.lo, s);
  }
  auto dgemm_pl = [&](const Img& A, const Planes& W, pfhip::PlaneGemmOp op) {
    const int N = op.N, K = op.K;
    Scope sc(m, s, K_GEMM, 2.0 * ML * (double)N * K, 4.0 * ((double)ML * K + (double)N * K + (double)ML * N));
    op.Ah = A.hi; op.Al = A.lo; op.rows_a = op.rows_p = MLp; op.Wh = W.hi; op.Wl = W.lo; op.rows_w = N; op.w_scale = W.scale;
    op.M = ML; op.ldr1 = d;
    pfhip::launch_gemm_p3(op, s);
  };
  auto dec_ffn = [&](const DecFfn& F, const float* xin, float* out) {
    if (dec_planes && xd_has_planes && xd_has_stats) {
      dgemm_pl(xdP, F.ffn1_f.img, {.C = m->hd.f(), .ldc = c.dec_ffn, .Ph = hdP.hi, .Pl = hdP.lo, .N = c.dec_ffn, .K = d, .bias = F.ffn1_f.folded.b,
                                   .relu = true, .ln_stats = m->lnstats.f(), .ln_tiles = 4, .ln_colsum = F.ffn1_f.colsum,
                                   .stats_out = m->lnstats2.f()});
      dgemm_pl(hdP, F.ffn2_f.img, {.C = out, .ldc = d, .N = d, .K = c.dec_ffn, .bias = F.ffn2_f.folded.b, .ln_stats = m->lnstats2.f(),
                                   .ln_tiles = ftiles, .ln_colsum = F.ffn2_f.colsum});
      return;
    }
    if (fuse_dec) {
      if (xd_has_stats) {
        x6ln(F.ffn1_f.folded, {.A = xin, .C = m->hd.f(), .N = c.dec_ffn, .K = d, .relu = true, .ln_stats = m->lnstats.f(), .ln_tiles = 4,
                               .ln_colsum = F.ffn1_f.colsum, .stats_out = m->lnstats2.f()});
      } else {
        lnorm(m, s, xin, d, m->yd.f(), d, F.norm1, ML, d, d);
        x6ln(F.ffn1, {.A = m->yd.f(), .C = m->hd.f(), .N = c.dec_ffn, .K = d, .relu = true, .stats_out = m->lnstats2.f()});
      }
      x6ln(F.ffn2_f.folded, {.A = m->hd.f(), .C = out, .N = d, .K = c.dec_ffn, .ln_stats = m->lnstats2.f(), .ln_tiles = ftiles,
                             .ln_colsum = F.ffn2_f.colsum});
      return;
    }
    lnorm(m, s, xin, d, m->yd.f(), d, F.norm1, ML, d, d);
    gemm(m, s, m->yd.f(), d, F.ffn1, c.dec_ffn, d, d, m->hd.f(), c.dec_ffn, nullptr, 0, nullptr, 0, ML, true);
    lnorm(m, s, m->hd.f(), c.dec_ffn, m->hd2.f(), c.dec_ffn, F.ffn_norm, ML, c.dec_ffn, c.dec_ffn);
    gemm(m, s, m->hd2.f(), c.dec_ffn, F.ffn2, d, c.dec_ffn, c.dec_ffn, out, d, nullptr, 0, nullptr, 0, ML, false);
  };
  auto cross_att = [&](const float* kv, const int* kv_off, const int* kv_len) {
    pfhip::AttnOp op = kv_attention(m->qd.f(), d, kv, 2 * d, m->ctxd.f());
    op.q_off = m->m_tok_off; op.q_len = m->m_tok_len; op.kv_off = kv_off; op.kv_len = kv_len;
    op.B = B; op.H = c.dec_n_head; op.max_q_len = m->maxL; op.scale = att_scale_d;
    return op;
  };
  for (int i = 0; i < c.dec_layers; ++i) {
    const DecLayer& L = w.dec[(size_t)i];
    dec_ffn(L.ffn, xd, m->td.f());
    lnorm(m, s, m->td.f(), d, m->t2.f(), d, L.norm2, ML, d, d);
    {
      Scope sc(m, s, K_FSMN, 2.0 * 11 * ML * d, 12.0 * ML * d);
      pfhip::launch_fsmn(m->t2.f(), d, L.fsmn_w, xd, d, xd, d, m->m_tok_off, m->m_tok_len, B, m->maxL, d, s);
    }
    lnorm(m, s, xd, d, m->yd.f(), d, L.norm3, ML, d, d);
    gemm(m, s, m->yd.f(), d, L.q, d, d, d, m->qd.f(), d, nullptr, 0, nullptr, 0, ML, false);
    const bool plain_layer = !(c.contextual && i == c.dec_layers - 1);
    if (side_kv) {
      kvbuf = m->kvside.f() + (size_t)i * Mp * 2 * d;
      HIP_TRY(hipStreamWaitEvent(s, m->ev_kv[(size_t)i], 0));
    } else if (dec_planes) {
      Scope sc(m, s, K_GEMM, 2.0 * M * 2.0 * d * d, 4.0 * ((double)M * d + 2.0 * d * d + 2.0 * M * d));
      const Planes& W = L.kv_img;
      pfhip::launch_gemm_p3({.Ah = encP.hi, .Al = encP.lo, .rows_a = Mp, .Wh = W.hi, .Wl = W.lo, .rows_w = 2 * d, .w_scale = W.scale, .C = kvbuf,
                             .ldc = 2 * d, .rows_p = Mp, .M = M, .N = 2 * d, .K = d, .bias = L.kv.b},
                            s);
    } else {
      gemm(m, s, m->enc.f(), d, L.kv, 2 * d, d, d, kvbuf, 2 * d, nullptr, 0, nullptr, 0, M, false);
    }
    {
      Scope sc(m, s, K_ATTN, 4.0 * cross_pairs * d, 8.0 * ML * d + 8.0 * M * d);
      pfhip::AttnOp att = cross_att(kvbuf, m->m_row_off, m->m_len);
      if (dec_planes && plain_layer) {
        att.planes_hi = ctxdP.hi; att.planes_lo = ctxdP.lo; att.plane_rows = MLp;
        pfhip::launch_attention_x3(att, s);
      } else {
        att.head_dim = hdd;
        pfhip::launch_attention(att, s);
      }
    }
    xd_has_stats = false;
    xd_has_planes = false;
    if (dec_planes && plain_layer) {
      dgemm_pl(ctxdP, L.out_img, {.C = xd, .ldc = d, .Ph = xdP.hi, .Pl = xdP.lo, .N = d, .K = d, .bias = L.out.b, .R1 = xd, .stats_out = m->lnstats.f()});
      xd_has_stats = true;
      xd_has_planes = true;
      continue;
    }
    if (plain_layer) {
      if (fuse_dec) {
        x6ln(L.out, {.A = m->ctxd.f(), .C = xd, .N = d, .K = d, .R1 = xd, .stats_out = m->lnstats.f()});
        xd_has_stats = true;
      } else {
        gemm(m, s, m->ctxd.f(), d, L.out, d, d, d, xd, d, xd, d, nullptr, 0, ML, false);
      }
      continue;
    }
    HIP_TRY(m->cat.ensure((size_t)MLp * 2 * d * 4));
    float* cat = m->cat.f();
    gemm(m, s, m->ctxd.f(), d, L.out, d, d, d, cat, 2 * d, nullptr, 0, nullptr, 0, ML, false);
    lnorm(m, s, xd, d, m->yd.f(), d, w.bias.norm3, ML, d, d);
    gemm(m, s, m->yd.f(), d, w.bias.q, d, d, d, m->qd.f(), d, nullptr, 0, nullptr, 0, ML, false);
    const float* hwkv = m->fw_hwkv;
    {
      double hw_pairs = 0;
      for (int b = 0; b < B; ++b) hw_pairs += (double)m->n_fires[b] * m->fw_hw_len[b];
      Scope sc(m, s, K_ATTN, 4.0 * hw_pairs * d, 8.0 * ML * d);
      pfhip::launch_attention(cross_att(hwkv, m->m_hw_off, m->m_hw_len), s);
    }
    gemm(m, s, m->ctxd.f(), d, w.bias.out, d, d, d, cat + d, 2 * d, nullptr, 0, nullptr, 0, ML, false);
    gemm(m, s, cat, 2 * d, w.bias.merge, d, 2 * d, 2 * d, xd, d, xd, d, nullptr, 0, ML, false);
  }
  dec_ffn(w.dec3, xd, m->td.f());
  lnorm(m, s, m->td.f(), d, m->yd.f(), d, w.dec_after, ML, d, d);
  gemm(m, s, m->yd.f(), d, w.dec_out, c.vocab, d, d, m->logits.f(), w.vocab_pad, nullptr, 0, nullptr, 0, ML, false);
  HIP_TRY(hipGetLastError());
  return PFHIP_OK;
}

pfhip_status ts_head_locked(pfhip_model* m, hipStream_t s, bool stepwise_only = false) {
  ForwardCtx fc(m);
  const Config& c = m->weights->cfg;
  const TimestampHead& ts = m->weights->ts;
  if (!c.timestamp) return fail(PFHIP_ERR_UNSUPPORTED, "model has no timestamp head (us_alphas / us_cif_peak outputs)");
  if (m->have_ts) return PFHIP_OK;
  const int d = c.d_model, B = m->B, M = m->M;
  if (M == 0) { m->have_ts = true; return PFHIP_OK; }
  const int Mp = round_up(M, pfhip::kTileM), R = 3 * M, Rp = 3 * Mp;
  HIP_TRY(m->ts_up.ensure((size_t)Rp * d * 4));
  HIP_TRY(m->ts_gx.ensure((size_t)Rp * 8 * d * 4));
  HIP_TRY(m->ts_y.ensure((size_t)Rp * 2 * d * 4));
  if (m->ts_hx.cap < (size_t)pfhip::kBlstmScratchFloats * 4) {
    HIP_TRY(m->ts_hx.ensure((size_t)pfhip::kBlstmScratchFloats * 4));
    HIP_TRY(hipMemsetAsync(m->ts_hx.p, 0, (size_t)pfhip::kBlstmScratchFloats * 4, s));
  }
  HIP_TRY(hipMemsetAsync(m->ts_hx.f() + pfhip::kBlstmFlagWord, 0, 4, s));
  if (m->debug_blstm_flag) {
    const unsigned one = 1u;
// ... 1630 lines not shown
```

### asr-2pass_amd/csrc/rowops.hip

```cpp
#include "kernels.h"

#include <math.h>

namespace pfhip {
namespace {

__device__ __forceinline__ float wave_sum(float v) {
#pragma unroll
  for (int off = 32; off >= 1; off >>= 1) v += __shfl_xor(v, off);
  return v;
}
__device__ __forceinline__ float wave_max(float v) {
#pragma unroll
  for (int off = 32; off >= 1; off >>= 1) v = fmaxf(v, __shfl_xor(v, off));
  return v;
}

template <int NV>
__global__ __launch_bounds__(256) void layernorm_kernel(const float* __restrict__ x, int ldx,
                                                        float* __restrict__ y, int ldy,
                                                        const float* __restrict__ g,
                                                        const float* __restrict__ b, int M, int D,
                                                        int Dout, float eps, int* range_flag) {
  const int wave = threadIdx.x >> 6, lane = threadIdx.x & 63;
// ... 11 lines not shown
  const float mean = wave_sum(s) / (float)D;
  float q = 0.f;
#pragma unroll
  for (int i = 0; i < NV; ++i) {
    const int c = (lane + 64 * i) * 4;
    if (c < D) {
      v[i].x -= mean; v[i].y -= mean; v[i].z -= mean; v[i].w -= mean;
      q += (v[i].x * v[i].x + v[i].y * v[i].y) + (v[i].z * v[i].z + v[i].w * v[i].w);
    }
  }
  const float rstd = 1.0f / sqrtf(wave_sum(q) / (float)D + eps);
  if (range_flag && lane == 0 && !(rstd < INFINITY)) atomicOr(range_flag, 1);
  float* yr = y + (size_t)row * ldy;
#pragma unroll
  for (int i = 0; i < NV; ++i) {
    const int c = (lane + 64 * i) * 4;
    if (c < D) {
      const float4 gg = *reinterpret_cast<const float4*>(g + c);
      const float4 bb = *reinterpret_cast<const float4*>(b + c);
      float4 o;
      o.x = v[i].x * rstd * gg.x + bb.x;
      o.y = v[i].y * rstd * gg.y + bb.y;
      o.z = v[i].z * rstd * gg.z + bb.z;
      o.w = v[i].w * rstd * gg.w + bb.w;
      *reinterpret_cast<float4*>(yr + c) = o;
    } else if (c < Dout) {
      *reinterpret_cast<float4*>(yr + c) = make_float4(0.f, 0.f, 0.f, 0.f);
    }
  }
}

constexpr int kFsmnK = 11;
constexpr int kTT = 16;

template <int LPAD>
__global__ __launch_bounds__(128) void fsmn_kernel(const float* __restrict__ v, int ldv,
                                                   const float* __restrict__ w,
                                                   const float* __restrict__ res, int ldres,
                                                   float* __restrict__ out, int ldo,
                                                   const int* __restrict__ off,
                                                   const int* __restrict__ len, int C) {
  const int b = blockIdx.y;
  const int L = len[b];
  const int t0 = blockIdx.x * kTT;
  if (t0 >= L) return;
  const int c = (blockIdx.z * 128 + threadIdx.x) * 4;
  if (c >= C) return;
  const size_t base = (size_t)off[b];
  float wk[4][kFsmnK];
#pragma unroll
  for (int ch = 0; ch < 4; ++ch)
#pragma unroll
    for (int j = 0; j < kFsmnK; ++j) wk[ch][j] = w[(size_t)(c + ch) * kFsmnK + j];

  constexpr int kHalf = LPAD;
  float4 rows[kTT + kFsmnK - 1];
#pragma unroll
  for (int j = 0; j < kTT + kFsmnK - 1; ++j) {
    const int t = t0 - kHalf + j;
    rows[j] = (t < 0 || t >= L) ? make_float4(0.f, 0.f, 0.f, 0.f) : *reinterpret_cast<const float4*>(v + (base + t) * ldv + c);
  }
  float4 rr[kTT];
  if (res) {
#pragma unroll
    for (int s = 0; s < kTT; ++s)
      rr[s] = (t0 + s < L) ? *reinterpret_cast<const float4*>(res + (base + t0 + s) * ldres + c) : make_float4(0.f, 0.f, 0.f, 0.f);
  }
#pragma unroll
  for (int s = 0; s < kTT; ++s) {
    const int t = t0 + s;
    if (t < L) {
      float4 o = rows[s + kHalf];
      if (res) { o.x += rr[s].x; o.y += rr[s].y; o.z += rr[s].z; o.w += rr[s].w; }
      float4 a = make_float4(0.f, 0.f, 0.f, 0.f);
#pragma unroll
      for (int j = 0; j < kFsmnK; ++j) {
        a.x += wk[0][j] * rows[s + j].x;
        a.y += wk[1][j] * rows[s + j].y;
        a.z += wk[2][j] * rows[s + j].z;
        a.w += wk[3][j] * rows[s + j].w;
      }
      o.x += a.x; o.y += a.y; o.z += a.z; o.w += a.w;
      *reinterpret_cast<float4*>(out + (base + t) * ldo + c) = o;
    }
  }
}

__global__ __launch_bounds__(128) void im2col3_kernel(const float* __restrict__ h, int ldh,
                                                      float* __restrict__ col, int ldc,
                                                      const int* __restrict__ row_pos,
                                                      const int* __restrict__ row_len, int M, int D) {
  const int row = blockIdx.x;
  if (row >= M) return;
  const int t = row_pos[row], L = row_len[row];
  for (int c4 = threadIdx.x; c4 < 3 * D / 4; c4 += blockDim.x) {
    const int c = c4 * 4;
    const int j = c / D, cc = c - j * D;
    const int tt = t + j - 1;
    float4 val = make_float4(0.f, 0.f, 0.f, 0.f);
    if (tt >= 0 && tt < L) val = *reinterpret_cast<const float4*>(h + (size_t)(row + j - 1) * ldh + cc);
    *reinterpret_cast<float4*>(col + (size_t)row * ldc + c) = val;
  }
}

__global__ __launch_bounds__(256) void alpha_kernel(const float* __restrict__ o, int ldo,
                                                    const float* __restrict__ w,
                                                    const float* __restrict__ b, float smooth,
                                                    float noise, float* __restrict__ alphas, int M,
                                                    int D) {
  const int wave = threadIdx.x >> 6, lane = threadIdx.x & 63;
  const int row = blockIdx.x * 4 + wave;
  if (row >= M) return;
  const float* orow = o + (size_t)row * ldo;
  float s = 0.f;
  for (int c = lane * 4; c < D; c += 256) {
    const float4 a = *reinterpret_cast<const float4*>(orow + c);
    const float4 ww = *reinterpret_cast<const float4*>(w + c);
    s += (a.x * ww.x + a.y * ww.y) + (a.z * ww.z + a.w * ww.w);
  }
  s = wave_sum(s) + b[0];
  if (lane == 0) {
    float a = 1.0f / (1.0f + expf(-s));
    a = fmaxf(a * smooth - noise, 0.f);
    alphas[row] = a;
  }
}

__global__ __launch_bounds__(256) void logsoftmax_argmax_kernel(const float* __restrict__ logits,
                                                                int ldl, int ML, int V,
                                                                float* __restrict__ logp,
                                                                int32_t* __restrict__ ids, int* range_flag) {
  __shared__ float s_max[4];
  __shared__ int s_idx[4];
  __shared__ float s_sum[4];
  const int row = blockIdx.x;
  if (row >= ML) return;
  const float* lr = logits + (size_t)row * ldl;
  const int wave = threadIdx.x >> 6, lane = threadIdx.x & 63;
  float best = -INFINITY;
  int bidx = 0x7fffffff;
  int bad = 0;
  if ((V & 3) == 0 && (ldl & 3) == 0) {
    for (int c4 = threadIdx.x; 4 * c4 < V; c4 += 256) {
      const float4 x = *reinterpret_cast<const float4*>(lr + 4 * c4);
      const int c = 4 * c4;
      if (x.x > best) { best = x.x; bidx = c; }
      if (x.y > best) { best = x.y; bidx = c + 1; }
      if (x.z > best) { best = x.z; bidx = c + 2; }
      if (x.w > best) { best = x.w; bidx = c + 3; }
      bad |= (int)!(fabsf(x.x) < INFINITY) | (int)!(fabsf(x.y) < INFINITY) | (int)!(fabsf(x.z) < INFINITY) | (int)!(fabsf(x.w) < INFINITY);
    }
  } else {
    for (int c = threadIdx.x; c < V; c += 256) {
      const float x = lr[c];
      if (x > best) { best = x; bidx = c; }
      bad |= (int)!(fabsf(x) < INFINITY);
    }
  }
#pragma unroll
  for (int off = 32; off >= 1; off >>= 1) {
    const float ob = __shfl_xor(best, off);
    const int oi = __shfl_xor(bidx, off);
    if (ob > best || (ob == best && oi < bidx)) { best = ob; bidx = oi; }
  }
  if (lane == 0) { s_max[wave] = best; s_idx[wave] = bidx; }
  __syncthreads();
// ... 18 lines not shown
    if (range_flag && !(fabsf(lse) < INFINITY)) atomicOr(range_flag, 1);
  }
  if (logp) {
    float* pr = logp + (size_t)row * V;
    for (int c = threadIdx.x; c < V; c += 256) pr[c] = (lr[c] - m) - lse;
  }
}

__global__ __launch_bounds__(128) void compact_kernel(const float* __restrict__ stage,
                                                      float* __restrict__ emb,
                                                      const int* __restrict__ src_row, int ML,
                                                      int D) {
  const int row = blockIdx.x;
  if (row >= ML) return;
  const float* s = stage + (size_t)src_row[row] * D;
  float* d = emb + (size_t)row * D;
  for (int c = threadIdx.x * 4; c < D; c += blockDim.x * 4)
    *reinterpret_cast<float4*>(d + c) = *reinterpret_cast<const float4*>(s + c);
}

__global__ __launch_bounds__(128) void gather_rows_kernel(const int32_t* __restrict__ ids,
                                                          const float* __restrict__ table, int D,
                                                          float* __restrict__ out, int R) {
  const int r = blockIdx.x;
  if (r >= R) return;
  const float* src = table + (size_t)ids[r] * D;
  for (int c = threadIdx.x * 4; c < D; c += blockDim.x * 4)
    *reinterpret_cast<float4*>(out + (size_t)r * D + c) = *reinterpret_cast<const float4*>(src + c);
}

__global__ __launch_bounds__(256) void lstm_cell_kernel(const float* __restrict__ G, float* __restrict__ c,
                                                        float* __restrict__ h, const int32_t* __restrict__ lens,
                                                        int t, float* __restrict__ sel, int H, int D) {
  const int j = blockIdx.x;
  if (j >= H) return;
  const float* g = G + (size_t)j * 4 * D;
  const bool pick = lens[j] - 1 == t;
  for (int k = threadIdx.x; k < D; k += blockDim.x) {
    const float ig = 1.0f / (1.0f + expf(-g[k]));
    const float fg = 1.0f / (1.0f + expf(-g[D + k]));
    const float gg = tanhf(g[2 * D + k]);
    const float og = 1.0f / (1.0f + expf(-g[3 * D + k]));
    const float cn = fg * c[(size_t)j * D + k] + ig * gg;
    const float hn = og * tanhf(cn);
    c[(size_t)j * D + k] = cn;
    h[(size_t)j * D + k] = hn;
    if (pick) sel[(size_t)j * D + k] = hn;
  }
}

}

void launch_gather_rows(const int32_t* ids, const float* table, int D, float* out, int R, hipStream_t s) {
  if (R <= 0) return;
  hipLaunchKernelGGL(gather_rows_kernel, dim3(R), dim3(128), 0, s, ids, table, D, out, R);
}

void launch_lstm_cell(const float* G, float* c, float* h, const int32_t* lens, int t, float* sel, int H, int D,
                      hipStream_t s) {
  if (H <= 0) return;
  hipLaunchKernelGGL(lstm_cell_kernel, dim3(H), dim3(256), 0, s, G, c, h, lens, t, sel, H, D);
}

void launch_layernorm(const float* x, int ldx, float* y, int ldy, const float* g, const float* b,
                      int M, int D, int Dout, float eps, hipStream_t s) {
  if (M <= 0) return;
  const dim3 grid((M + 3) / 4), block(256);
  const int nv = (Dout + 255) / 256;
  if (nv <= 2)
    hipLaunchKernelGGL(layernorm_kernel<2>, grid, block, 0, s, x, ldx, y, ldy, g, b, M, D, Dout, eps, launch_ctx().range_flag);
  else if (nv <= 3)
    hipLaunchKernelGGL(layernorm_kernel<3>, grid, block, 0, s, x, ldx, y, ldy, g, b, M, D, Dout, eps, launch_ctx().range_flag);
  else
    hipLaunchKernelGGL(layernorm_kernel<8>, grid, block, 0, s, x, ldx, y, ldy, g, b, M, D, Dout, eps, launch_ctx().range_flag);
}

void launch_fsmn(const float* v, int ldv, const float* w, const float* res, int ldres, float* out,
                 int ldo, const int* off, const int* len, int B, int max_len, int C, hipStream_t s) {
  if (B <= 0 || max_len <= 0) return;
  const dim3 grid((max_len + kTT - 1) / kTT, B, (C + 511) / 512), block(128);
  hipLaunchKernelGGL(fsmn_kernel<5>, grid, block, 0, s, v, ldv, w, res, ldres, out, ldo, off, len, C);
}

void launch_fsmn_shift(const float* v, int ldv, const float* w, const float* res, int ldres, float* out, int ldo,
                       const int* off, const int* len, int B, int max_len, int C, int shift, hipStream_t s) {
  if (B <= 0 || max_len <= 0) return;
  const dim3 grid((max_len + kTT - 1) / kTT, B, (C + 511) / 512), block(128);
  if (shift == 5)
    hipLaunchKernelGGL(fsmn_kernel<10>, grid, block, 0, s, v, ldv, w, res, ldres, out, ldo, off, len, C);
  else
    hipLaunchKernelGGL(fsmn_kernel<5>, grid, block, 0, s, v, ldv, w, res, ldres, out, ldo, off, len, C);
}

void launch_im2col3(const float* h, int ldh, float* col, int ldc, const int* row_pos,
                    const int* row_len, int M, int D, hipStream_t s) {
  if (M <= 0) return;
  hipLaunchKernelGGL(im2col3_kernel, dim3(M), dim3(128), 0, s, h, ldh, col, ldc, row_pos, row_len, M, D);
}

void launch_alpha(const float* o, int ldo, const float* w, const float* b, float smooth, float noise,
                  float* alphas, int M, int D, hipStream_t s) {
  if (M <= 0) return;
  hipLaunchKernelGGL(alpha_kernel, dim3((M + 3) / 4), dim3(256), 0, s, o, ldo, w, b, smooth, noise,
                     alphas, M, D);
}

void launch_compact(const float* stage, float* emb, const int* tok_row_src, int ML, int D,
                    hipStream_t s) {
  if (ML <= 0) return;
  hipLaunchKernelGGL(compact_kernel, dim3(ML), dim3(128), 0, s, stage, emb, tok_row_src, ML, D);
}

void launch_logsoftmax_argmax(const float* logits, int ldl, int ML, int V, float* logp, int32_t* ids,
                              hipStream_t s, int* range_flag) {
  if (ML <= 0) return;
  hipLaunchKernelGGL(logsoftmax_argmax_kernel, dim3(ML), dim3(256), 0, s, logits, ldl, ML, V, logp, ids, range_flag);
}

}
```

### asr-2pass_amd/ops.py

```python
from __future__ import annotations

import ctypes

import torch

from . import load_lib, PfhipError

_vp, _ci, _cf = ctypes.c_void_p, ctypes.c_int, ctypes.c_float
_bound = False


def _lib():
    global _bound
    lib = load_lib()
    if not _bound:
        lib.pfhip_op_gemm_f32.argtypes = [_vp, _ci, _vp, _ci, _vp, _ci, _vp, _vp, _ci, _vp, _ci, _ci, _ci, _ci, _ci, _ci, _vp]
        lib.pfhip_op_gemm_f32_kind.argtypes = [_vp, _ci, _vp, _ci, _vp, _ci, _vp, _vp, _ci, _vp, _ci, _ci, _ci, _ci, _ci, _ci, _ci, _vp]
        lib.pfhip_op_fused_ln_gemm.argtypes = [_vp, _ci, _ci, _vp, _vp, _cf, _vp, _ci, _vp, _ci, _vp, _vp, _ci, _vp, _ci, _vp, _ci, _vp,
                                               _ci, _ci, _ci, _ci, _vp]
        lib.pfhip_op_fused_gemv_1trip.argtypes = [_vp, _ci, _vp, _ci, _vp, _ci, _vp, _vp, _cf, _vp, _ci, _vp, _ci, _vp, _ci, _ci, _ci, _ci, _vp]
        lib.pfhip_op_window_attention.argtypes = [_vp, _ci, _vp, _ci, _vp, _ci, _vp, _ci, _ci, _ci, _ci, _cf, _vp]
        lib.pfhip_op_window_attention_hd.argtypes = [_vp, _ci, _vp, _ci, _vp, _ci, _vp, _ci, _ci, _ci, _ci, _cf, _ci, _vp]
        lib.pfhip_op_fused_att_out.argtypes = [_vp, _ci, _vp, _ci, _vp, _ci, _ci, _ci, _ci, _cf, _vp, _ci, _vp, _ci, _vp, _vp, _ci, _vp, _ci, _vp,
                                               _ci, _vp]
# ... 86 lines not shown
                w_scale=1.0, out=None):
    lib = _lib()
    K = A.shape[1]
    M = A.shape[0] if M is None else M
    N = W.shape[0] if N is None else N
    if out is None:
        out = torch.empty((round_up(M, 128), N), dtype=torch.float32, device=A.device)
    if w_scale == "auto":
        w_scale = best_w_scale(float(W.abs().max()))
    lib.pfhip_op_gemm_f32_ln.argtypes = [_vp, _ci, _vp, _ci, _vp, _ci, _vp, _vp, _ci, _vp, _ci, _ci, _ci, _ci, _ci, _vp, _ci, _vp, _vp,
                                         ctypes.c_float, _vp]
    _ck(lib.pfhip_op_gemm_f32_ln(_p(A), A.stride(0), _p(W), W.stride(0), _p(out), out.stride(0), _p(bias), _p(R1),
                                 R1.stride(0) if R1 is not None else 0, _p(R2), R2.stride(0) if R2 is not None else 0, M, N, K,
                                 1 if relu else 0, _p(ln_stats), ln_tiles, _p(ln_colsum), _p(stats_out), float(w_scale), _stream()),
        "gemm_f32_ln")
    return out


def fused_ln_gemm(X, W, M, N, g=None, b=None, D=None, bias=None, R1=None, R2=None, fsmn_v=None, fsmn_w=None, relu=False, out=None,
                  eps=1e-12):
    K = W.shape[1]
    if out is None:
        out = torch.zeros((32, round_up(N, 128)), dtype=torch.float32, device=X.device)
    _ck(_lib().pfhip_op_fused_ln_gemm(_p(X), X.stride(0), K if D is None else D, _p(g), _p(b), eps, _p(W), W.stride(0), _p(out),
                                      out.stride(0), _p(bias), _p(R1), R1.stride(0) if R1 is not None else 0, _p(R2),
                                      R2.stride(0) if R2 is not None else 0, _p(fsmn_v), fsmn_v.stride(0) if fsmn_v is not None else 0,
                                      _p(fsmn_w), M, N, K, 1 if relu else 0, _stream()), "fused_ln_gemm")
    return out


def fold_layernorm(W, bias, g, b):
    Wd = W.double()
    Wf = (Wd * g.double()[None, :]).float()
    bf = ((bias.double() if bias is not None else 0.0) + Wd @ b.double()).float()
    return Wf, bf, Wf.double().sum(1).float()


def fused_gemv_1trip(X, W, M, N, bias=None, ln_colsum=None, R1=None, fsmn_v=None, fsmn_w=None, relu=False, out=None, eps=1e-12):
    K = W.shape[1]
    if out is None:
        out = torch.zeros((32, round_up(N, 128)), dtype=torch.float32, device=X.device)
    _ck(_lib().pfhip_op_fused_gemv_1trip(_p(X), X.stride(0), _p(W), W.stride(0), _p(out), out.stride(0), _p(bias), _p(ln_colsum), eps,
                                         _p(R1), R1.stride(0) if R1 is not None else 0, _p(fsmn_v),
                                         fsmn_v.stride(0) if fsmn_v is not None else 0, _p(fsmn_w), M, N, K, 1 if relu else 0, _stream()),
        "fused_gemv_1trip")
    return out


def fused_gemv_1trip_route(M, N, K, ln=False, fsmn=False):
    lib = _lib()
    lib.pfhip_op_fused_gemv_1trip_route.argtypes = [_ci, _ci, _ci, _ci, _ci, ctypes.POINTER(_ci)]
    out = (_ci * 8)()
    _ck(lib.pfhip_op_fused_gemv_1trip_route(int(M), int(N), int(K), 1 if ln else 0, 1 if fsmn else 0, out), "fused_gemv_1trip_route")
    ok, ln_, fs, cw, cpl, rpl, nf, waves = list(out)
    return dict(ok=bool(ok), ln=bool(ln_), fs=bool(fs), cw=cw, cpl=cpl, rpl=rpl, nf=nf, waves=waves)


def fused_ln_gemm_route(M, N, K, ln=False):
    lib = _lib()
    lib.pfhip_op_fused_ln_gemm_route.argtypes = [_ci, _ci, _ci, _ci, ctypes.POINTER(_ci)]
    out = (_ci * 6)()
    _ck(lib.pfhip_op_fused_ln_gemm_route(int(M), int(N), int(K), 1 if ln else 0, out), "fused_ln_gemm_route")
    kernel, ln_, cw, mr, waves, k_blocks = list(out)
    return dict(kernel={1: "vector", 2: "matrix"}.get(kernel, "none"), ln=bool(ln_), cw=cw, mr=mr, waves=waves, k_blocks=k_blocks)


def layernorm(x, g, b, D=None, Dout=None, eps=1e-12):
    M = x.shape[0]
    D = x.shape[1] if D is None else D
    Dout = D if Dout is None else Dout
    y = torch.empty((M, Dout), dtype=torch.float32, device=x.device)
    _ck(_lib().pfhip_op_layernorm(_p(x), x.stride(0), _p(y), y.stride(0), _p(g), _p(b), M, D, Dout, eps, _stream()), "layernorm")
    return y


def fsmn(v, w, off, length, res=None):
    out = torch.zeros((v.shape[0], v.shape[1]), dtype=torch.float32, device=v.device)
    B = off.numel()
    _ck(_lib().pfhip_op_fsmn(_p(v), v.stride(0), _p(w), _p(res), res.stride(0) if res is not None else 0, _p(out),
                             out.stride(0), _p(off), _p(length), B, int(length.max().item()), v.shape[1], _stream()), "fsmn")
    return out


def fsmn_shift(v, w, off, length, shift, res=None):
    lib = _lib()
    lib.pfhip_op_fsmn_shift.argtypes = [_vp, _ci, _vp, _vp, _ci, _vp, _ci, _vp, _vp, _ci, _ci, _ci, _ci, _vp]
    out = torch.zeros((v.shape[0], v.shape[1]), dtype=torch.float32, device=v.device)
    _ck(lib.pfhip_op_fsmn_shift(_p(v), v.stride(0), _p(w), _p(res), res.stride(0) if res is not None else 0, _p(out), out.stride(0),
                                _p(off), _p(length), off.numel(), int(length.max().item()), v.shape[1], int(shift), _stream()),
        "fsmn_shift")
    return out


def resample(x, in_off, n_in, fs_in, fs_out=16000):
    import numpy as np
    from . import resample_len
    n_in = [int(v) for v in n_in]
    n_out = [resample_len(fs_in, v, fs_out) for v in n_in]
    if any(v < 0 for v in n_out):
        raise PfhipError(f"unsupported rate pair {fs_in} -> {fs_out}")
    out_off = np.zeros(len(n_in), np.int64)
    out_off[1:] = np.cumsum(n_out[:-1]) if len(n_in) > 1 else out_off[1:]
    y = torch.empty(max(sum(n_out), 1), dtype=torch.float32, device=x.device)
    io = np.ascontiguousarray(in_off, np.int64)
    ni = np.ascontiguousarray(n_in, np.int32)
    _ck(_lib().pfhip_op_resample(_p(x), ctypes.c_void_p(io.ctypes.data), ctypes.c_void_p(ni.ctypes.data), len(n_in), fs_in, fs_out,
                                 _p(y), ctypes.c_void_p(out_off.ctypes.data), _stream()), "resample")
    return y, [int(v) for v in out_off], n_out


def attention(Q, K, V, q_off, q_len, kv_off, kv_len, n_head, scale, head_dim=128):
    O = torch.zeros((Q.shape[0], n_head * head_dim), dtype=torch.float32, device=Q.device)
    B = q_off.numel()
    _ck(_lib().pfhip_op_attention_hd(_p(Q), Q.stride(0), _p(K), K.stride(0), _p(V), V.stride(0), _p(O), O.stride(0),
                                     _p(q_off), _p(q_len), _p(kv_off), _p(kv_len), B, n_head, int(q_len.max().item()),
                                     scale, head_dim, _stream()), "attention")
    return O


def attention_limit(Q, K, V, q_off, q_len, kv_off, kv_len, n_head, scale, q_kv_limit, head_dim=128):
    lib = _lib()
    lib.pfhip_op_attention_limit.argtypes = [_vp, _ci, _vp, _ci, _vp, _ci, _vp, _ci, _vp, _vp, _vp, _vp, _ci, _ci, _ci, _cf, _ci, _vp, _vp]
    O = torch.zeros((Q.shape[0], n_head * head_dim), dtype=torch.float32, device=Q.device)
    _ck(lib.pfhip_op_attention_limit(_p(Q), Q.stride(0), _p(K), K.stride(0), _p(V), V.stride(0), _p(O), O.stride(0), _p(q_off), _p(q_len),
                                     _p(kv_off), _p(kv_len), q_off.numel(), n_head, int(q_len.max().item()), float(scale), int(head_dim),
                                     _p(q_kv_limit), _stream()), "attention_limit")
    return O


def attention_dk(Q, K, V, q_off, q_len, kv_off, kv_len, n_head, scale, d_k, q_kv_limit=None, out=None):
    lib = _lib()
    O = torch.zeros((Q.shape[0], n_head * d_k), dtype=torch.float32, device=Q.device) if out is None else out
    _ck(lib.pfhip_op_attention_dk(_p(Q), Q.stride(0), _p(K), K.stride(0), _p(V), V.stride(0), _p(O), O.stride(0),
                                  _p(q_off), _p(q_len), _p(kv_off), _p(kv_len), q_off.numel(), n_head, int(q_len.max().item()),
                                  float(scale), int(d_k), _p(q_kv_limit), _stream()), "attention_dk")
    return O


def attention_fsmn_is_fused(max_len, head_dim=128):
    lib = _lib()
    lib.pfhip_op_attention_fsmn_is_fused.argtypes = [_ci, _ci]
    return bool(lib.pfhip_op_attention_fsmn_is_fused(int(max_len), int(head_dim)))


def attention_fsmn(Q, K, V, off, length, n_head, scale, fsmn_w, mem, mem_accumulate=False, head_dim=128):
    lib = _lib()
    O = torch.zeros((Q.shape[0], n_head * head_dim), dtype=torch.float32, device=Q.device)
    lib.pfhip_op_attention_fsmn.argtypes = [_vp, _ci, _vp, _ci, _vp, _ci, _vp, _ci, _vp, _vp, _ci, _ci, _ci, _cf, _vp, _vp, _ci, _ci, _ci, _vp]
    _ck(lib.pfhip_op_attention_fsmn(_p(Q), Q.stride(0), _p(K), K.stride(0), _p(V), V.stride(0), _p(O), O.stride(0), _p(off), _p(length),
                                    off.numel(), n_head, int(length.max().item()), float(scale), _p(fsmn_w), _p(mem), mem.stride(0),
                                    1 if mem_accumulate else 0, head_dim, _stream()), "attention_fsmn")
    return O


def attention_planes(Q, K, V, q_off, q_len, kv_off, kv_len, n_head, scale):
    lib = _lib()
    rows = round_up(Q.shape[0], 128)
    lib.pfhip_op_plane_image_bytes.restype = ctypes.c_size_t
    lib.pfhip_op_plane_image_bytes.argtypes = [_ci, _ci]
    nb = int(lib.pfhip_op_plane_image_bytes(rows, n_head * 128))
    hi = torch.zeros(nb, dtype=torch.uint8, device=Q.device)
    lo = torch.zeros(nb, dtype=torch.uint8, device=Q.device)
    lib.pfhip_op_attention_planes.argtypes = [_vp, _ci, _vp, _ci, _vp, _ci, _vp, _vp, _ci, _vp, _vp, _vp, _vp, _ci, _ci, _ci, _ci,
                                             ctypes.c_float, _vp]
    _ck(lib.pfhip_op_attention_planes(_p(Q), Q.stride(0), _p(K), K.stride(0), _p(V), V.stride(0), _p(hi), _p(lo), rows, _p(q_off),
                                      _p(q_len), _p(kv_off), _p(kv_len), q_off.numel(), n_head, int(q_len.max().item()), Q.shape[0],
# ... 144 lines not shown
    V = W.shape[0] if V is None else V
    if E is None:
        E = torch.empty(max(lab.e_floats, 1), dtype=torch.float32, device=X.device)
    e_off = lab.e_off + int(e_base)
    _ck(_lib().pfhip_op_ctc_emissions(_p(X), X.stride(0), _p(W), W.stride(0), _p(bias), _p(lse), _p(row_off), _p(lab.len), _p(lab.lab_off),
                                      _p(lab.n_lab), _p(lab.labels), _p(e_off), lab.B, X.shape[1], V, int(blank), _p(E), _stream()),
        "ctc_emissions")
    return E


def ctc_align_workspace_bytes(e_floats):
    return int(_lib().pfhip_op_ctc_align_workspace_bytes(int(e_floats)))


def ctc_align(E, lab, max_tokens=None, want_logp=True, workspace_bytes=None):
    lib = _lib()
    max_tokens = max(lab.n + [0]) if max_tokens is None else int(max_tokens)
    if any(n > max_tokens for n in lab.n):
        raise PfhipError("ctc_align: an utterance has more labels than max_tokens")
    dev = lab.len.device
    tok_begin = torch.full((lab.B, max(max_tokens, 1)), -7, dtype=torch.int32, device=dev)
    tok_end = torch.full((lab.B, max(max_tokens, 1)), -7, dtype=torch.int32, device=dev)
    tok_logp = torch.full((lab.B, max(max_tokens, 1)), float("nan"), dtype=torch.float32, device=dev) if want_logp else None
    score = torch.full((max(lab.B, 1),), float("nan"), dtype=torch.float32, device=dev)
    nbytes = ctc_align_workspace_bytes(lab.e_floats) if workspace_bytes is None else int(workspace_bytes)
    ws = torch.empty(max(nbytes, 1), dtype=torch.uint8, device=dev)
    _ck(lib.pfhip_op_ctc_align(_p(E), _p(lab.e_off), lab.e_floats, _p(lab.len), _p(lab.n_lab), _p(lab.labels), _p(lab.lab_off), lab.B,
                               max_tokens, _p(tok_begin), _p(tok_end), _p(tok_logp), _p(score), _p(ws), nbytes, _stream()), "ctc_align")
    return tok_begin[:, :max_tokens], tok_end[:, :max_tokens], None if tok_logp is None else tok_logp[:, :max_tokens], score[:lab.B]


def split_planes(X, rows=None, scale=1.0, rows_valid=None):
    lib = _lib()
    R, K = X.shape
    rows_valid = R if rows_valid is None else rows_valid
    rows = round_up(R if rows is None else rows, 128)
    lib.pfhip_op_plane_image_bytes.restype = ctypes.c_size_t
    lib.pfhip_op_plane_image_bytes.argtypes = [_ci, _ci]
    nb = int(lib.pfhip_op_plane_image_bytes(rows, K))
    hi = torch.empty(nb, dtype=torch.uint8, device=X.device)
    lo = torch.empty(nb, dtype=torch.uint8, device=X.device)
    lib.pfhip_op_split_planes.argtypes = [_vp, _ci, _ci, _ci, _ci, ctypes.c_float, _vp, _vp, _vp]
    _ck(lib.pfhip_op_split_planes(_p(X), X.stride(0), rows_valid, rows, K, float(scale), _p(hi), _p(lo), _stream()), "split_planes")
    return hi, lo, rows


def planes_to_float(hi, lo, rows, K):
    import numpy as np
    out = np.zeros((rows, K), np.float64)
    for img in (hi, lo):
        a = img.cpu().numpy().view(np.float16).reshape(K // 16, rows, 2, 8).astype(np.float64)
        swap = ((np.arange(rows) >> 3) & 1).astype(bool)
        a[:, swap] = a[:, swap][:, :, ::-1]
        out += a.transpose(1, 0, 2, 3).reshape(rows, K)
    return out


def gemm_p3(A_img, W_img, M, N, K, w_scale=1.0, bias=None, R1=None, relu=False, want_c=True, want_planes=False, ln_stats=None,
            ln_tiles=0, ln_colsum=None, stats_out=None, out=None, out_planes=None, tile_rows=0, tile_cols=0):
    lib = _lib()
    ah, al, ra = A_img
    wh, wl, rw = W_img
    Mp = round_up(M, 128)
    C = (out if out is not None else torch.empty((Mp, N), dtype=torch.float32, device=ah.device)) if want_c else None
    P = None
    if want_planes and out_planes is not None:
        P = out_planes
    elif want_planes:
        nb = int(lib.pfhip_op_plane_image_bytes(Mp, N))
        P = (torch.zeros(nb, dtype=torch.uint8, device=ah.device), torch.zeros(nb, dtype=torch.uint8, device=ah.device), Mp)
    lib.pfhip_op_gemm_p3.argtypes = [_vp, _vp, _ci, _vp, _vp, _ci, ctypes.c_float, _vp, _ci, _vp, _vp, _ci, _vp, _vp, _ci, _ci, _ci, _ci, _ci,
                                     _vp, _ci, _vp, _vp, _ci, _vp]
    args = (_p(ah), _p(al), ra, _p(wh), _p(wl), rw, float(w_scale), _p(C), N if want_c else 0, _p(P[0]) if P else None,
            _p(P[1]) if P else None, Mp, _p(bias), _p(R1), R1.stride(0) if R1 is not None else 0, M, N, K,
            1 if relu else 0, _p(ln_stats), ln_tiles, _p(ln_colsum), _p(stats_out), tile_rows)
    if tile_cols:
        lib.pfhip_op_gemm_p3_cols.argtypes = lib.pfhip_op_gemm_p3.argtypes[:-1] + [_ci, _vp]
        _ck(lib.pfhip_op_gemm_p3_cols(*args, tile_cols, _stream()), "gemm_p3")
    else:
        _ck(lib.pfhip_op_gemm_p3(*args, _stream()), "gemm_p3")
    return C, P


def gemm_p3_wide_launches():
    lib = _lib()
    lib.pfhip_op_gemm_p3_wide_launches.restype = ctypes.c_long
    return int(lib.pfhip_op_gemm_p3_wide_launches())


def split_rows(X, ldp=None, out=None, col=0):
    lib = _lib()
    R, C = X.shape
    ldp = C if ldp is None else ldp
    if out is None:
        out = (torch.zeros((R, ldp), dtype=torch.float16, device=X.device), torch.zeros((R, ldp), dtype=torch.float16, device=X.device))
    hi, lo = out
    lib.pfhip_op_split_rows.argtypes = [_vp, _ci, _ci, _ci, _vp, _vp, _ci, _vp]
    _ck(lib.pfhip_op_split_rows(_p(X), X.stride(0), R, C, hi.data_ptr() + 2 * col, lo.data_ptr() + 2 * col, ldp, _stream()), "split_rows")
    return hi, lo


def gemm_p3_qkv(A_img, W_img, M, N, K, q_cols, w_scale=1.0, bias=None, ln_stats=None, ln_tiles=0, ln_colsum=None, tile_rows=0):
    lib = _lib()
    ah, al, ra = A_img
    wh, wl, rw = W_img
    Mp = round_up(M, 128)
    C = torch.zeros((Mp, q_cols), dtype=torch.float32, device=ah.device)
    kvh = torch.zeros((Mp, N - q_cols), dtype=torch.float16, device=ah.device)
    kvl = torch.zeros((Mp, N - q_cols), dtype=torch.float16, device=ah.device)
    lib.pfhip_op_gemm_p3_qkv.argtypes = [_vp, _vp, _ci, _vp, _vp, _ci, ctypes.c_float, _vp, _ci, _vp, _vp, _ci, _ci, _vp, _ci, _ci, _ci, _vp, _ci,
                                         _vp, _ci, _vp]
    _ck(lib.pfhip_op_gemm_p3_qkv(_p(ah), _p(al), ra, _p(wh), _p(wl), rw, float(w_scale), _p(C), q_cols, _p(kvh), _p(kvl), N - q_cols, q_cols,
                                 _p(bias), M, N, K, _p(ln_stats), ln_tiles, _p(ln_colsum), tile_rows, _stream()), "gemm_p3_qkv")
    return C, (kvh, kvl)


def attention_kvplanes(Q, kv, v_col, q_off, q_len, kv_off, kv_len, n_head, scale, fsmn_w=None, mem=None, mem_accumulate=False,
                       want_planes=False):
    lib = _lib()
    kvh, kvl = kv
    O, P = None, None
    rows = round_up(Q.shape[0], 128)
    if want_planes:
        lib.pfhip_op_plane_image_bytes.restype = ctypes.c_size_t
        lib.pfhip_op_plane_image_bytes.argtypes = [_ci, _ci]
        nb = int(lib.pfhip_op_plane_image_bytes(rows, n_head * 128))
        P = (torch.zeros(nb, dtype=torch.uint8, device=Q.device), torch.zeros(nb, dtype=torch.uint8, device=Q.device), rows)
    else:
        O = torch.zeros((Q.shape[0], n_head * 128), dtype=torch.float32, device=Q.device)
    lib.pfhip_op_attention_kvplanes.argtypes = [_vp, _ci, _vp, _vp, _ci, _ci, _ci, _vp, _ci, _vp, _vp, _ci, _vp, _vp, _vp, _vp, _ci, _ci, _ci, _ci,
                                                ctypes.c_float, _vp, _vp, _ci, _ci, _vp]
    _ck(lib.pfhip_op_attention_kvplanes(_p(Q), Q.stride(0), _p(kvh), _p(kvl), kvh.stride(0), v_col, kvh.shape[0], _p(O),
                                        O.stride(0) if O is not None else 0, _p(P[0]) if P else None, _p(P[1]) if P else None, rows,
                                        _p(q_off), _p(q_len), _p(kv_off), _p(kv_len), q_off.numel(), n_head, int(q_len.max().item()),
                                        Q.shape[0], float(scale), _p(fsmn_w), _p(mem), mem.stride(0) if mem is not None else 0,
                                        1 if mem_accumulate else 0, _stream()), "attention_kvplanes")
    return P if want_planes else O


def _hi(values):
    import numpy as np
    a = np.ascontiguousarray(values, np.int32)
    return a, ctypes.c_void_p(a.ctypes.data)


_ll = ctypes.c_longlong


def cif_stream(enc, alphas, row_off, n, is_last, pre, suf, carry, D, threshold, tail, emb, n_fire):
    B = len(n)
    lib = _lib()
    lib.pfhip_op_cif_stream.argtypes = [_vp, _ci, _vp, _vp, _vp, _vp, _vp, _vp, _vp, _ll, _ci, _ci, _cf, _cf, _vp, _ci, _vp, _vp]
    ro, n_, il, pr, su = _hi(row_off), _hi(n), _hi(is_last), _hi(pre), _hi(suf)
    _ck(lib.pfhip_op_cif_stream(_p(enc), enc.stride(0), _p(alphas), ro[1], n_[1], il[1], pr[1], su[1], _p(carry), carry.stride(0), B, D,
                                float(threshold), float(tail), _p(emb), emb.shape[1], _p(n_fire), _stream()), "cif_stream")


def cif_stream_fires(enc, alphas, row_off, n, is_last, pre, suf, carry, D, threshold, tail, emb, n_fire, fire_step):
    B = len(n)
    lib = _lib()
    lib.pfhip_op_cif_stream_fires.argtypes = [_vp, _ci, _vp, _vp, _vp, _vp, _vp, _vp, _vp, _ll, _ci, _ci, _cf, _cf, _vp, _ci, _vp, _vp, _vp]
    ro, n_, il, pr, su = _hi(row_off), _hi(n), _hi(is_last), _hi(pre), _hi(suf)
    _ck(lib.pfhip_op_cif_stream_fires(_p(enc), enc.stride(0), _p(alphas), ro[1], n_[1], il[1], pr[1], su[1], _p(carry), carry.stride(0), B,
                                      D, float(threshold), float(tail), _p(emb), emb.shape[1], _p(n_fire), _p(fire_step), _stream()),
        "cif_stream_fires")

# ... 110 lines not shown
```

### include/pfhip_ops.h

```cpp
#ifndef PFHIP_OPS_H_
#define PFHIP_OPS_H_
#include <stdint.h>
#ifdef __cplusplus
extern "C" {
#endif

int pfhip_op_gemm_f32(const float* A, int lda, const float* W, int ldw, float* C, int ldc, const float* bias,
                      const float* R1, int ldr1, const float* R2, int ldr2, int M, int N, int K, int relu,
                      int guard, void* stream);
int pfhip_op_gemm_f32_kind(const float* A, int lda, const float* W, int ldw, float* C, int ldc, const float* bias,
                           const float* R1, int ldr1, const float* R2, int ldr2, int M, int N, int K, int relu,
                           int guard, int kind, void* stream);
int pfhip_op_gemm_f32_scaled(const float* A, int lda, const float* W, int ldw, float* C, int ldc, const float* bias,
                             const float* R1, int ldr1, const float* R2, int ldr2, int M, int N, int K, int relu,
                             int guard, int kind, float w_scale, void* stream);
float pfhip_op_best_w_scale(float max_abs);
int pfhip_op_set_launch_ctx(int* range_flag, int exact);
int pfhip_op_gemm_f32_ln(const float* A, int lda, const float* W, int ldw, float* C, int ldc, const float* bias, const float* R1, int ldr1,
                         const float* R2, int ldr2, int M, int N, int K, int relu, const float* ln_stats, int ln_tiles,
                         const float* ln_colsum, float* stats_out, float w_scale, void* stream);
size_t pfhip_op_plane_image_bytes(int rows, int K);
int pfhip_op_split_planes(const float* X, int ld, int rows_valid, int rows, int K, float scale, void* hi, void* lo, void* stream);
int pfhip_op_gemm_p3(const void* Ah, const void* Al, int rows_a, const void* Wh, const void* Wl, int rows_w, float w_scale, float* C, int ldc,
                     void* Ph, void* Pl, int rows_p, const float* bias, const float* R1, int ldr1, int M, int N, int K, int relu,
                     const float* ln_stats, int ln_tiles, const float* ln_colsum, float* stats_out, int tile_rows, void* stream);
int pfhip_op_gemm_p3_cols(const void* Ah, const void* Al, int rows_a, const void* Wh, const void* Wl, int rows_w, float w_scale, float* C, int ldc,
                          void* Ph, void* Pl, int rows_p, const float* bias, const float* R1, int ldr1, int M, int N, int K, int relu,
                          const float* ln_stats, int ln_tiles, const float* ln_colsum, float* stats_out, int tile_rows, int tile_cols,
                          void* stream);
long pfhip_op_gemm_p3_wide_launches(void);
int pfhip_op_layernorm(const float* x, int ldx, float* y, int ldy, const float* g, const float* b, int M, int D,
                       int Dout, float eps, void* stream);
int pfhip_op_fsmn(const float* v, int ldv, const float* w, const float* res, int ldres, float* out, int ldo,
                  const int* off, const int* len, int B, int max_len, int C, void* stream);
int pfhip_op_fsmn_shift(const float* v, int ldv, const float* w, const float* res, int ldres, float* out, int ldo,
                        const int* off, const int* len, int B, int max_len, int C, int shift, void* stream);
int pfhip_op_attention(const float* Q, int ldq, const float* K, int ldk, const float* V, int ldv, float* O, int ldo,
                       const int* q_off, const int* q_len, const int* kv_off, const int* kv_len, int B, int H,
                       int max_q_len, float scale, void* stream);
int pfhip_op_attention_hd(const float* Q, int ldq, const float* K, int ldk, const float* V, int ldv, float* O, int ldo,
                          const int* q_off, const int* q_len, const int* kv_off, const int* kv_len, int B, int H,
                          int max_q_len, float scale, int head_dim, void* stream);
int pfhip_op_attention_limit(const float* Q, int ldq, const float* K, int ldk, const float* V, int ldv, float* O, int ldo,
                             const int* q_off, const int* q_len, const int* kv_off, const int* kv_len, int B, int H,
                             int max_q_len, float scale, int head_dim, const int* q_kv_limit, void* stream);
int pfhip_op_attention_dk(const float* Q, int ldq, const float* K, int ldk, const float* V, int ldv, float* O, int ldo,
                          const int* q_off, const int* q_len, const int* kv_off, const int* kv_len, int B, int H,
                          int max_q_len, float scale, int d_k, const int* q_kv_limit, void* stream);
int pfhip_op_attention_fsmn(const float* Q, int ldq, const float* K, int ldk, const float* V, int ldv, float* O, int ldo, const int* off,
                            const int* len, int B, int H, int max_len, float scale, const float* fsmn_w, float* mem, int ldmem,
                            int mem_accumulate, int head_dim, void* stream);
int pfhip_op_attention_fsmn_is_fused(int max_len, int head_dim);
int pfhip_op_attention_planes(const float* Q, int ldq, const float* K, int ldk, const float* V, int ldv, void* planes_hi, void* planes_lo,
                              int plane_rows, const int* q_off, const int* q_len, const int* kv_off, const int* kv_len, int B, int H,
                              int max_q_len, int total_q_rows, float scale, void* stream);
int pfhip_op_split_rows(const float* X, int ld, int rows, int cols, void* hi, void* lo, int ldp, void* stream);
int pfhip_op_gemm_p3_qkv(const void* Ah, const void* Al, int rows_a, const void* Wh, const void* Wl, int rows_w, float w_scale, float* C, int ldc,
                         void* kv_hi, void* kv_lo, int ldkv, int q_cols, const float* bias, int M, int N, int K, const float* ln_stats,
                         int ln_tiles, const float* ln_colsum, int tile_rows, void* stream);
int pfhip_op_attention_kvplanes(const float* Q, int ldq, const void* kv_hi, const void* kv_lo, int ldkv, int v_col, int total_kv_rows, float* O,
                                int ldo, void* planes_hi, void* planes_lo, int plane_rows, const int* q_off, const int* q_len,
                                const int* kv_off, const int* kv_len, int B, int H, int max_q_len, int total_q_rows, float scale,
                                const float* fsmn_w, float* mem, int ldmem, int mem_accumulate, void* stream);
int pfhip_op_cif(const float* hidden, int ldh, const float* alphas, const int* row_off, const int* len, int B, int D,
                 float threshold, float tail, float* stage, int* n_fires, int* token_num, void* stream);
int pfhip_op_cif_fires(const float* hidden, int ldh, const float* alphas, const int* row_off, const int* len, int B, int D,
                       float threshold, float tail, float* stage, int* n_fires, int* token_num, int* fire_frame, void* stream);
int pfhip_op_logsoftmax_argmax(const float* logits, int ldl, int ML, int V, float* logp, int32_t* ids, void* stream);
int pfhip_op_logsoftmax_topk(const float* logits, int ldl, int M, int V, int k, float* logp, int32_t* ids, int32_t* topk_ids,
                             float* topk_logp, void* stream);

size_t pfhip_op_ctc_head_workspace_bytes(int M, int V);
int pfhip_op_ctc_head(const float* X, int ldx, const float* W, int ldw, const float* bias, float w_scale, int M, int V, int K,
                      int32_t* ids, float* logp_best, float* lse, void* workspace, size_t workspace_bytes, void* stream);
int pfhip_op_ctc_collapse(const int32_t* frame_ids, const float* frame_logp, const int* row_off, const int* len, int B, int blank,
                          int max_tokens, int32_t* ids, int32_t* tok_frame, float* tok_logp, int32_t* token_num, void* stream);
int pfhip_op_ctc_collapse_chunk(void);
int pfhip_op_ctc_emissions(const float* X, int ldx, const float* W, int ldw, const float* bias, const float* lse, const int* row_off,
                           const int* len, const int* lab_off, const int* n_lab, const int32_t* labels, const long long* e_off, int B,
                           int K, int V, int blank, float* E, void* stream);
size_t pfhip_op_ctc_align_workspace_bytes(size_t e_floats);
int pfhip_op_ctc_align_max_tokens(void);
int pfhip_op_ctc_align(const float* E, const long long* e_off, size_t e_floats, const int* len, const int* n_lab, const int32_t* labels,
                       const int* lab_off, int B, int max_tokens, int32_t* tok_begin, int32_t* tok_end, float* tok_logp, float* score,
                       void* workspace, size_t workspace_bytes, void* stream);
int pfhip_op_fused_ln_gemm(const float* X, int ldx, int D, const float* g, const float* b, float eps, const float* W, int ldw,
                           float* C, int ldc, const float* bias, const float* R1, int ldr1, const float* R2, int ldr2,
                           const float* fsmn_v, int ldv, const float* fsmn_w, int M, int N, int K, int relu, void* stream);

int pfhip_op_fused_gemv_1trip(const float* X, int ldx, const float* W, int ldw, float* C, int ldc, const float* bias,
                              const float* ln_colsum, float eps, const float* R1, int ldr1, const float* fsmn_v, int ldv,
                              const float* fsmn_w, int M, int N, int K, int relu, void* stream);
int pfhip_op_fused_gemv_1trip_route(int M, int N, int K, int has_ln, int has_fsmn, int* out);
int pfhip_op_fused_ln_gemm_route(int M, int N, int K, int has_ln, int* out);

int pfhip_op_window_attention(const float* Q, int ldq, const float* K, int ldk, const float* V, int ldv, float* O, int ldo, int Lq, int Lk,
                              int H, float scale, void* stream);
int pfhip_op_window_attention_hd(const float* Q, int ldq, const float* K, int ldk, const float* V, int ldv, float* O, int ldo, int Lq, int Lk,
                                 int H, float scale, int head_dim, void* stream);
int pfhip_op_window_attention_segments(const float* Q, int ldq, const float* K, int ldk, const float* V, int ldv, float* O, int ldo,
                                       const int* q_off, const int* q_len, const int* kv_off, const int* kv_len, int B, int H, int max_q_len,
                                       int max_kv_len, float scale, const float* fsmn_w, float* mem, int ldmem, int head_dim, void* stream);

int pfhip_op_fused_att_out(const float* Q, int ldq, const float* K, int ldk, const float* V, int ldv, int Lq, int Lk, int H, float scale,
                           const float* W, int ldw, float* C, int ldc, const float* bias, const float* R1, int ldr1, const float* fsmn_v,
                           int ldfv, const float* fsmn_w, int N, void* stream);

int pfhip_op_resample_table(int fs_in, int fs_out, int32_t* first_index, int32_t* ntaps, float* weights, size_t cap_floats,
                            int* n_phases, int* taps, int* in_unit);
int pfhip_op_resample(const float* d_in, const int64_t* in_off, const int* n_in, int batch, int fs_in, int fs_out, float* d_out,
                      const int64_t* out_off, void* stream);

int pfhip_op_cif_stream(const float* enc, int lde, const float* alphas, const int* row_off, const int* n, const int* is_last,
                        const int* pre, const int* suf, float* carry, long long carry_stride, int B, int D, float threshold,
                        float tail, float* emb, int emb_rows, int* n_fire, void* stream);
int pfhip_op_cif_stream_fires(const float* enc, int lde, const float* alphas, const int* row_off, const int* n, const int* is_last,
                              const int* pre, const int* suf, float* carry, long long carry_stride, int B, int D, float threshold,
// ... 28 lines not shown
```

Measured before the change: 40610.

## Skip fp32 store of decoder FFN1 output and add fused LN-FSMN-LN row kernel

The decoder FFN1 GEMM now writes only the fp16 plane image plus row statistics and no longer stores the fp32 hidden matrix. The GEMM epilogue gains null checks on C, and a stats-only output mode is added. Separately, a new kernel fuses norm2, the FSMN memory block with its residual, and norm3 into one launch by staging normalized rows in LDS, which removes two intermediate global round trips. The fused kernel is gated behind the PFHIP_DEC_ROWCHAIN environment variable, which is off by default, so only the FFN1 store removal runs by default.

```diff
diff --git a/asr-2pass_amd/csrc/gemm_p3.hip b/asr-2pass_amd/csrc/gemm_p3.hip
--- a/asr-2pass_amd/csrc/gemm_p3.hip
+++ b/asr-2pass_amd/csrc/gemm_p3.hip
@@ -309,7 +309,7 @@
       }
       v.x += e_bv.x + e_r1[pass].x; v.y += e_bv.y + e_r1[pass].y; v.z += e_bv.z + e_r1[pass].z; v.w += e_bv.w + e_r1[pass].w;
       if (relu) { v.x = fmaxf(v.x, 0.f); v.y = fmaxf(v.y, 0.f); v.z = fmaxf(v.z, 0.f); v.w = fmaxf(v.w, 0.f); }
-      if (do_store && grow < M && e_cols) *reinterpret_cast<float4*>(C + (size_t)grow * ldc + gcol) = v;
+      if (do_store && C && grow < M && e_cols) *reinterpret_cast<float4*>(C + (size_t)grow * ldc + gcol) = v;
       if (OUT & 2) *reinterpret_cast<float4*>(Cs + row * kPCs + 4 * c4) = v;
       if (stats_out) tile_row_stats(v, grow, M, tn, tiles_n, c4, stats_out);
     }
@@ -516,7 +516,7 @@
         }
         v.x += bv.x + r1v[pass].x; v.y += bv.y + r1v[pass].y; v.z += bv.z + r1v[pass].z; v.w += bv.w + r1v[pass].w;
         if (relu) { v.x = fmaxf(v.x, 0.f); v.y = fmaxf(v.y, 0.f); v.z = fmaxf(v.z, 0.f); v.w = fmaxf(v.w, 0.f); }
-        if (grow < M && gcol + 3 < N) *reinterpret_cast<float4*>(C + (size_t)grow * ldc + gcol) = v;
+        if (C && grow < M && gcol + 3 < N) *reinterpret_cast<float4*>(C + (size_t)grow * ldc + gcol) = v;
         if (OUT & 2) *reinterpret_cast<float4*>(Cs + row * kPCs + 4 * c4) = v;
         if (stats_out) tile_row_stats(v, grow, M, tn, tiles_n, c4, stats_out);
       }
@@ -600,7 +600,7 @@
       }
       v.x += bv.x + r1v[pass].x; v.y += bv.y + r1v[pass].y; v.z += bv.z + r1v[pass].z; v.w += bv.w + r1v[pass].w;
       if (relu) { v.x = fmaxf(v.x, 0.f); v.y = fmaxf(v.y, 0.f); v.z = fmaxf(v.z, 0.f); v.w = fmaxf(v.w, 0.f); }
-      if (grow < M && gcol + 3 < N) *reinterpret_cast<float4*>(C + (size_t)grow * ldc + gcol) = v;
+      if (C && grow < M && gcol + 3 < N) *reinterpret_cast<float4*>(C + (size_t)grow * ldc + gcol) = v;
       if (OUT & 2) *reinterpret_cast<float4*>(Cs + row * kPCs + 4 * c4) = v;
       if (stats_out) tile_row_stats(v, grow, M, tn, tiles_n, c4, stats_out);
     }
@@ -1243,7 +1243,7 @@
   const int n_tiles = ((M + tmr - 1) / tmr) * tiles_n;
   static const int gw_env = env_int("PFHIP_P3_GW", 0);
   const int gw = std::max(1, std::min(gw_env > 0 ? gw_env : kGroupWidth, tiles_n));
-  const int out = (C ? 1 : 0) | (ph ? 2 : 0);
+  const int out = (C || o.stats_out ? 1 : 0) | (ph ? 2 : 0);
 #define PFHIP_P3_GO(THREADS, LDS, ...)                                                                                                        \
   launch_with_lds<__VA_ARGS__, THREADS>(n_tiles, LDS, s, ah, al, rows_a, wh, wl, o.rows_w, C, o.ldc, ph, pl, o.rows_p, o.bias, o.R1, o.ldr1, M, N, K, \
                                         tiles_n, n_tiles, gw, rl, o.ln_stats, o.ln_tiles, 1e-12f, o.ln_colsum, o.stats_out, inv,              \
diff --git a/asr-2pass_amd/csrc/kernels.h b/asr-2pass_amd/csrc/kernels.h
--- a/asr-2pass_amd/csrc/kernels.h
+++ b/asr-2pass_amd/csrc/kernels.h
@@ -102,6 +102,9 @@
 
 void launch_fsmn(const float* v, int ldv, const float* w, const float* res, int ldres, float* out,
                  int ldo, const int* off, const int* len, int B, int max_len, int C, hipStream_t s);
+bool dec_rowchain_serves(int D);
+void launch_dec_rowchain(const float* td, const float* g2, const float* b2, const float* w, float* xd, const float* g3, const float* b3,
+                         float* yd, const int* off, const int* len, int B, int max_len, int D, float eps, hipStream_t s);
 void launch_fsmn_shift(const float* v, int ldv, const float* w, const float* res, int ldres, float* out,
                        int ldo, const int* off, const int* len, int B, int max_len, int C, int shift, hipStream_t s);
 
diff --git a/asr-2pass_amd/csrc/ops_abi.cpp b/asr-2pass_amd/csrc/ops_abi.cpp
--- a/asr-2pass_amd/csrc/ops_abi.cpp
+++ b/asr-2pass_amd/csrc/ops_abi.cpp
@@ -161,13 +161,14 @@
   pfhip::launch_split_planes(X, ld, rows_valid, rows, K, scale, hi, lo, S(stream));
   return (int)hipGetLastError();
 }
-int pfhip_op_gemm_p3(const void* Ah, const void* Al, int rows_a, const void* Wh, const void* Wl, int rows_w, float w_scale, float* C, int ldc,
-                     void* Ph, void* Pl, int rows_p, const float* bias, const float* R1, int ldr1, int M, int N, int K, int relu,
-                     const float* ln_stats, int ln_tiles, const float* ln_colsum, float* stats_out, int tile_rows, void* stream) {
+namespace {
+int op_gemm_p3(const void* Ah, const void* Al, int rows_a, const void* Wh, const void* Wl, int rows_w, float w_scale, float* C, int ldc,
+               void* Ph, void* Pl, int rows_p, const float* bias, const float* R1, int ldr1, int M, int N, int K, int relu,
+               const float* ln_stats, int ln_tiles, const float* ln_colsum, float* stats_out, int tile_rows, bool stats_without_c, void* stream) {
   const int mp = (M + 127) / 128 * 128;
   if (M <= 0 || N <= 0 || K < 16 || K % 16 || N % 128 || rows_a % 128 || rows_w % 128 || rows_a < mp || rows_w < N || !Ah || !Al || !Wh ||
       !Wl || (!C && !Ph) || (Ph && (!Pl || rows_p % 128 || rows_p < mp)) || (C && ldc < N) || (R1 && ldr1 < N) || !(w_scale > 0.f) ||
-      (ln_stats && (!ln_colsum || ln_tiles <= 0)) || (stats_out && !C)  ||
+      (ln_stats && (!ln_colsum || ln_tiles <= 0)) || (stats_out && !C && !stats_without_c) ||
       (tile_rows != 0 && tile_rows != 64 && tile_rows != 128 && tile_rows != 256))
     return (int)hipErrorInvalidValue;
   pfhip::launch_gemm_p3({.Ah = Ah, .Al = Al, .rows_a = rows_a, .Wh = Wh, .Wl = Wl, .rows_w = rows_w, .w_scale = w_scale, .C = C, .ldc = ldc,
@@ -175,6 +176,20 @@
                          .relu = relu != 0, .ln_stats = ln_stats, .ln_tiles = ln_tiles, .ln_colsum = ln_colsum, .stats_out = stats_out},
                         S(stream), tile_rows);
   return (int)hipGetLastError();
+}
+}
+int pfhip_op_gemm_p3(const void* Ah, const void* Al, int rows_a, const void* Wh, const void* Wl, int rows_w, float w_scale, float* C, int ldc,
+                     void* Ph, void* Pl, int rows_p, const float* bias, const float* R1, int ldr1, int M, int N, int K, int relu,
+                     const float* ln_stats, int ln_tiles, const float* ln_colsum, float* stats_out, int tile_rows, void* stream) {
+  return op_gemm_p3(Ah, Al, rows_a, Wh, Wl, rows_w, w_scale, C, ldc, Ph, Pl, rows_p, bias, R1, ldr1, M, N, K, relu, ln_stats, ln_tiles, ln_colsum,
+                    stats_out, tile_rows, false, stream);
+}
+int pfhip_op_gemm_p3_planes_stats(const void* Ah, const void* Al, int rows_a, const void* Wh, const void* Wl, int rows_w, float w_scale, void* Ph,
+                                  void* Pl, int rows_p, const float* bias, const float* R1, int ldr1, int M, int N, int K, int relu,
+                                  const float* ln_stats, int ln_tiles, const float* ln_colsum, float* stats_out, int tile_rows, void* stream) {
+  if (!Ph || !stats_out) return (int)hipErrorInvalidValue;
+  return op_gemm_p3(Ah, Al, rows_a, Wh, Wl, rows_w, w_scale, nullptr, 0, Ph, Pl, rows_p, bias, R1, ldr1, M, N, K, relu, ln_stats, ln_tiles,
+                    ln_colsum, stats_out, tile_rows, true, stream);
 }
 int pfhip_op_gemm_p3_cols(const void* Ah, const void* Al, int rows_a, const void* Wh, const void* Wl, int rows_w, float w_scale, float* C, int ldc,
                           void* Ph, void* Pl, int rows_p, const float* bias, const float* R1, int ldr1, int M, int N, int K, int relu,
@@ -206,6 +221,12 @@
                   const int* off, const int* len, int B, int max_len, int C, void* stream) {
   if (C % 4) return (int)hipErrorInvalidValue;
   pfhip::launch_fsmn(v, ldv, w, res, ldres, out, ldo, off, len, B, max_len, C, S(stream));
+  return done();
+}
+int pfhip_op_dec_rowchain(const float* td, const float* g2, const float* b2, const float* w, float* xd, const float* g3, const float* b3,
+                          float* yd, const int* off, const int* len, int B, int max_len, int D, float eps, void* stream) {
+  if (!pfhip::dec_rowchain_serves(D) || !td || !g2 || !b2 || !w || !xd || !g3 || !b3 || !yd || !off || !len) return (int)hipErrorInvalidValue;
+  pfhip::launch_dec_rowchain(td, g2, b2, w, xd, g3, b3, yd, off, len, B, max_len, D, eps, S(stream));
   return done();
 }
 int pfhip_op_fsmn_shift(const float* v, int ldv, const float* w, const float* res, int ldres, float* out, int ldo,
diff --git a/asr-2pass_amd/csrc/pfhip.cpp b/asr-2pass_amd/csrc/pfhip.cpp
--- a/asr-2pass_amd/csrc/pfhip.cpp
+++ b/asr-2pass_amd/csrc/pfhip.cpp
@@ -1002,10 +1002,10 @@
   HIP_TRY(m->emb.ensure((size_t)MLp * d * 4));
   HIP_TRY(m->xd.ensure((size_t)MLp * d * 4));
   HIP_TRY(m->yd.ensure((size_t)MLp * d * 4));
-  HIP_TRY(m->hd.ensure((size_t)MLp * c.dec_ffn * 4));
-  HIP_TRY(m->hd2.ensure((size_t)MLp * c.dec_ffn * 4));
   HIP_TRY(m->td.ensure((size_t)MLp * d * 4));
-  HIP_TRY(m->t2.ensure((size_t)MLp * d * 4));
+  static const bool rowchain_env = pfhip::env_on("PFHIP_DEC_ROWCHAIN");
+  const bool rowchain = rowchain_env && pfhip::dec_rowchain_serves(d);
+  if (!rowchain) HIP_TRY(m->t2.ensure((size_t)MLp * d * 4));
   HIP_TRY(m->qd.ensure((size_t)MLp * d * 4));
   HIP_TRY(m->ctxd.ensure((size_t)MLp * d * 4));
   HIP_TRY(m->logits.ensure((size_t)MLp * w.vocab_pad * 4));
@@ -1037,6 +1037,8 @@
   const float att_scale_d = 1.0f / sqrtf((float)hdd);
   const bool fuse_dec = w.dec_folded && pfhip::gemm_x6_ln_ok(ML) && !pfhip::launch_ctx().exact;
   const int ftiles = c.dec_ffn / pfhip::kTileN;
+  HIP_TRY(m->hd.ensure((size_t)MLp * c.dec_ffn * 4));
+  if (!fuse_dec) HIP_TRY(m->hd2.ensure((size_t)MLp * c.dec_ffn * 4));
   if (fuse_dec) {
     HIP_TRY(m->lnstats.ensure((size_t)std::max(Mp, MLp) * 4 * 2 * 4));
     HIP_TRY(m->lnstats2.ensure((size_t)MLp * ftiles * 2 * 4));
@@ -1073,7 +1075,7 @@
   };
   auto dec_ffn = [&](const DecFfn& F, const float* xin, float* out) {
     if (dec_planes && xd_has_planes && xd_has_stats) {
-      dgemm_pl(xdP, F.ffn1_f.img, {.C = m->hd.f(), .ldc = c.dec_ffn, .Ph = hdP.hi, .Pl = hdP.lo, .N = c.dec_ffn, .K = d, .bias = F.ffn1_f.folded.b,
+      dgemm_pl(xdP, F.ffn1_f.img, {.Ph = hdP.hi, .Pl = hdP.lo, .N = c.dec_ffn, .K = d, .bias = F.ffn1_f.folded.b,
                                    .relu = true, .ln_stats = m->lnstats.f(), .ln_tiles = 4, .ln_colsum = F.ffn1_f.colsum,
                                    .stats_out = m->lnstats2.f()});
       dgemm_pl(hdP, F.ffn2_f.img, {.C = out, .ldc = d, .N = d, .K = c.dec_ffn, .bias = F.ffn2_f.folded.b, .ln_stats = m->lnstats2.f(),
@@ -1106,12 +1108,18 @@
   for (int i = 0; i < c.dec_layers; ++i) {
     const DecLayer& L = w.dec[(size_t)i];
     dec_ffn(L.ffn, xd, m->td.f());
-    lnorm(m, s, m->td.f(), d, m->t2.f(), d, L.norm2, ML, d, d);
-    {
-      Scope sc(m, s, K_FSMN, 2.0 * 11 * ML * d, 12.0 * ML * d);
-      pfhip::launch_fsmn(m->t2.f(), d, L.fsmn_w, xd, d, xd, d, m->m_tok_off, m->m_tok_len, B, m->maxL, d, s);
-    }
-    lnorm(m, s, xd, d, m->yd.f(), d, L.norm3, ML, d, d);
+    if (rowchain) {
+      Scope sc(m, s, K_FSMN, (2.0 * 11 + 16.0) * ML * d, 16.0 * ML * d);
+      pfhip::launch_dec_rowchain(m->td.f(), L.norm2.g, L.norm2.b, L.fsmn_w, xd, L.norm3.g, L.norm3.b, m->yd.f(), m->m_tok_off, m->m_tok_len, B,
+                                 m->maxL, d, 1e-12f, s);
+    } else {
+      lnorm(m, s, m->td.f(), d, m->t2.f(), d, L.norm2, ML, d, d);
+      {
+        Scope sc(m, s, K_FSMN, 2.0 * 11 * ML * d, 12.0 * ML * d);
+        pfhip::launch_fsmn(m->t2.f(), d, L.fsmn_w, xd, d, xd, d, m->m_tok_off, m->m_tok_len, B, m->maxL, d, s);
+      }
+      lnorm(m, s, xd, d, m->yd.f(), d, L.norm3, ML, d, d);
+    }
     gemm(m, s, m->yd.f(), d, L.q, d, d, d, m->qd.f(), d, nullptr, 0, nullptr, 0, ML, false);
     const bool plain_layer = !(c.contextual && i == c.dec_layers - 1);
     if (side_kv) {
diff --git a/asr-2pass_amd/csrc/rowops.hip b/asr-2pass_amd/csrc/rowops.hip
--- a/asr-2pass_amd/csrc/rowops.hip
+++ b/asr-2pass_amd/csrc/rowops.hip
@@ -117,6 +117,175 @@
       }
       o.x += a.x; o.y += a.y; o.z += a.z; o.w += a.w;
       *reinterpret_cast<float4*>(out + (base + t) * ldo + c) = o;
+    }
+  }
+}
+
+constexpr int kRcT = 16;
+constexpr int kRcRows = kRcT + kFsmnK - 1;
+constexpr int kRcThreads = 512;
+constexpr int kRcWaves = kRcThreads / 64;
+constexpr int kRcP1 = (kRcRows + kRcWaves - 1) / kRcWaves;
+constexpr int kRcNV = 2;
+
+template <int NV>
+__device__ __forceinline__ float rc_center(float4 (&v)[NV], int lane, int D, float eps, int* range_flag) {
+  float s = 0.f;
+#pragma unroll
+  for (int i = 0; i < NV; ++i) s += (v[i].x + v[i].y) + (v[i].z + v[i].w);
+  const float mean = wave_sum(s) / (float)D;
+  float q = 0.f;
+#pragma unroll
+  for (int i = 0; i < NV; ++i) {
+    const int c = (lane + 64 * i) * 4;
+    if (c < D) {
+      v[i].x -= mean; v[i].y -= mean; v[i].z -= mean; v[i].w -= mean;
+      q += (v[i].x * v[i].x + v[i].y * v[i].y) + (v[i].z * v[i].z + v[i].w * v[i].w);
+    }
+  }
+  const float rstd = 1.0f / sqrtf(wave_sum(q) / (float)D + eps);
+  if (range_flag && lane == 0 && !(rstd < INFINITY)) atomicOr(range_flag, 1);
+  return rstd;
+}
+
+__global__ __launch_bounds__(kRcThreads, 4) void dec_rowchain_kernel(const float* __restrict__ td, const float* __restrict__ g2,
+                                                                    const float* __restrict__ b2, const float* __restrict__ w,
+                                                                    float* xd, const float* __restrict__ g3,
+                                                                    const float* __restrict__ b3, float* __restrict__ yd,
+                                                                    const int* __restrict__ off, const int* __restrict__ len, int D,
+                                                                    float eps, int* range_flag) {
+  extern __shared__ __attribute__((aligned(16))) float rc_rows[];
+  const int b = blockIdx.y;
+  const int L = len[b];
+  const int t0 = blockIdx.x * kRcT;
+  if (t0 >= L) return;
+  const size_t base = (size_t)off[b];
+  const int tid = threadIdx.x, wave = tid >> 6, lane = tid & 63;
+
+  constexpr int kOwn = kRcT / (kRcThreads / 256);
+  const int c = (tid & 255) * 2, s0 = (tid >> 8) * kOwn;
+  const bool owner = c < D;
+  float2 rr[kOwn];
+  if (owner) {
+#pragma unroll
+    for (int s = 0; s < kOwn; ++s)
+      rr[s] = (t0 + s0 + s < L) ? *reinterpret_cast<const float2*>(xd + (base + t0 + s0 + s) * D + c) : make_float2(0.f, 0.f);
+  }
+
+  {
+    float4 v[kRcP1][kRcNV];
+#pragma unroll
+    for (int p = 0; p < kRcP1; ++p) {
+      const int t = t0 - 5 + wave + kRcWaves * p;
+      const bool in = wave + kRcWaves * p < kRcRows && t >= 0 && t < L;
+#pragma unroll
+      for (int i = 0; i < kRcNV; ++i) {
+        const int cc = (lane + 64 * i) * 4;
+        v[p][i] = (in && cc < D) ? *reinterpret_cast<const float4*>(td + (base + t) * D + cc) : make_float4(0.f, 0.f, 0.f, 0.f);
+      }
+    }
+    float4 gg[kRcNV], bb[kRcNV];
+#pragma unroll
+    for (int i = 0; i < kRcNV; ++i) {
+      const int cc = (lane + 64 * i) * 4;
+      gg[i] = cc < D ? *reinterpret_cast<const float4*>(g2 + cc) : make_float4(0.f, 0.f, 0.f, 0.f);
+      bb[i] = cc < D ? *reinterpret_cast<const float4*>(b2 + cc) : make_float4(0.f, 0.f, 0.f, 0.f);
+    }
+#pragma unroll
+    for (int p = 0; p < kRcP1; ++p) {
+      const int j = wave + kRcWaves * p, t = t0 - 5 + j;
+      if (j >= kRcRows) continue;
+      float* lr = rc_rows + j * D;
+      if (t >= 0 && t < L) {
+        const float rstd = rc_center<kRcNV>(v[p], lane, D, eps, range_flag);
+#pragma unroll
+        for (int i = 0; i < kRcNV; ++i) {
+          const int cc = (lane + 64 * i) * 4;
+          if (cc < D) {
+            float4 o;
+            o.x = v[p][i].x * rstd * gg[i].x + bb[i].x;
+            o.y = v[p][i].y * rstd * gg[i].y + bb[i].y;
+            o.z = v[p][i].z * rstd * gg[i].z + bb[i].z;
+            o.w = v[p][i].w * rstd * gg[i].w + bb[i].w;
+            *reinterpret_cast<float4*>(lr + cc) = o;
+          }
+        }
+      } else {
+#pragma unroll
+        for (int i = 0; i < kRcNV; ++i) {
+          const int cc = (lane + 64 * i) * 4;
+          if (cc < D) *reinterpret_cast<float4*>(lr + cc) = make_float4(0.f, 0.f, 0.f, 0.f);
+        }
+      }
+    }
+  }
+  float wk[2][kFsmnK];
+  if (owner) {
+#pragma unroll
+    for (int ch = 0; ch < 2; ++ch)
+#pragma unroll
+      for (int j = 0; j < kFsmnK; ++j) wk[ch][j] = w[(size_t)(c + ch) * kFsmnK + j];
+  }
+  __syncthreads();
+
+  float2 rows[kOwn + kFsmnK - 1];
+  if (owner) {
+#pragma unroll
+    for (int j = 0; j < kOwn + kFsmnK - 1; ++j) rows[j] = *reinterpret_cast<const float2*>(rc_rows + (s0 + j) * D + c);
+  }
+  __syncthreads();
+  if (owner) {
+#pragma unroll
+    for (int s = 0; s < kOwn; ++s) {
+      if (t0 + s0 + s < L) {
+        float2 o = rows[s + 5];
+        o.x += rr[s].x; o.y += rr[s].y;
+        float2 a = make_float2(0.f, 0.f);
+#pragma unroll
+        for (int j = 0; j < kFsmnK; ++j) {
+          a.x += wk[0][j] * rows[s + j].x;
+          a.y += wk[1][j] * rows[s + j].y;
+        }
+        o.x += a.x; o.y += a.y;
+        *reinterpret_cast<float2*>(xd + (base + t0 + s0 + s) * D + c) = o;
+        *reinterpret_cast<float2*>(rc_rows + (s0 + s + 5) * D + c) = o;
+      }
+    }
+  }
+  __syncthreads();
+
+  {
+    float4 gg[kRcNV], bb[kRcNV];
+#pragma unroll
+    for (int i = 0; i < kRcNV; ++i) {
+      const int cc = (lane + 64 * i) * 4;
+      gg[i] = cc < D ? *reinterpret_cast<const float4*>(g3 + cc) : make_float4(0.f, 0.f, 0.f, 0.f);
+      bb[i] = cc < D ? *reinterpret_cast<const float4*>(b3 + cc) : make_float4(0.f, 0.f, 0.f, 0.f);
+    }
+#pragma unroll
+    for (int p = 0; p < kRcT / kRcWaves; ++p) {
+      const int s = wave + kRcWaves * p, t = t0 + s;
+      if (t >= L) continue;
+      float4 v[kRcNV];
+#pragma unroll
+      for (int i = 0; i < kRcNV; ++i) {
+        const int cc = (lane + 64 * i) * 4;
+        v[i] = cc < D ? *reinterpret_cast<const float4*>(rc_rows + (s + 5) * D + cc) : make_float4(0.f, 0.f, 0.f, 0.f);
+      }
+      const float rstd = rc_center<kRcNV>(v, lane, D, eps, range_flag);
+      float* yr = yd + (base + t) * D;
+#pragma unroll
+      for (int i = 0; i < kRcNV; ++i) {
+        const int cc = (lane + 64 * i) * 4;
+        if (cc < D) {
+          float4 o;
+          o.x = v[i].x * rstd * gg[i].x + bb[i].x;
+          o.y = v[i].y * rstd * gg[i].y + bb[i].y;
+          o.z = v[i].z * rstd * gg[i].z + bb[i].z;
+          o.w = v[i].w * rstd * gg[i].w + bb[i].w;
+          *reinterpret_cast<float4*>(yr + cc) = o;
+        }
+      }
     }
   }
 }
@@ -301,6 +470,15 @@
   hipLaunchKernelGGL(fsmn_kernel<5>, grid, block, 0, s, v, ldv, w, res, ldres, out, ldo, off, len, C);
 }
 
+bool dec_rowchain_serves(int D) { return D > 0 && D % 4 == 0 && D <= 256 * kRcNV; }
+void launch_dec_rowchain(const float* td, const float* g2, const float* b2, const float* w, float* xd, const float* g3, const float* b3,
+                         float* yd, const int* off, const int* len, int B, int max_len, int D, float eps, hipStream_t s) {
+  if (B <= 0 || max_len <= 0) return;
+  const dim3 grid((max_len + kRcT - 1) / kRcT, B), block(kRcThreads);
+  hipLaunchKernelGGL(dec_rowchain_kernel, grid, block, (size_t)kRcRows * D * sizeof(float), s, td, g2, b2, w, xd, g3, b3, yd, off, len, D, eps,
+                     launch_ctx().range_flag);
+}
+
 void launch_fsmn_shift(const float* v, int ldv, const float* w, const float* res, int ldres, float* out, int ldo,
                        const int* off, const int* len, int B, int max_len, int C, int shift, hipStream_t s) {
   if (B <= 0 || max_len <= 0) return;
diff --git a/asr-2pass_amd/ops.py b/asr-2pass_amd/ops.py
--- a/asr-2pass_amd/ops.py
+++ b/asr-2pass_amd/ops.py
@@ -192,6 +192,17 @@
     return out
 
 
+def dec_rowchain(td, g2, b2, w, xd, g3, b3, off, length, eps=1e-12):
+    lib = _lib()
+    lib.pfhip_op_dec_rowchain.argtypes = [_vp, _vp, _vp, _vp, _vp, _vp, _vp, _vp, _vp, _vp, _ci, _ci, _ci, _cf, _vp]
+    if not (td.is_contiguous() and xd.is_contiguous() and td.shape == xd.shape):
+        raise PfhipError("dec_rowchain needs dense td / xd of one shape")
+    yd = torch.zeros_like(xd)
+    _ck(lib.pfhip_op_dec_rowchain(_p(td), _p(g2), _p(b2), _p(w), _p(xd), _p(g3), _p(b3), _p(yd), _p(off), _p(length), off.numel(),
+                                  int(length.max().item()), td.shape[1], eps, _stream()), "dec_rowchain")
+    return yd
+
+
 def fsmn_shift(v, w, off, length, shift, res=None):
     lib = _lib()
     lib.pfhip_op_fsmn_shift.argtypes = [_vp, _ci, _vp, _vp, _ci, _vp, _ci, _vp, _vp, _ci, _ci, _ci, _ci, _vp]
@@ -502,6 +513,24 @@
     return C, P
 
 
+def gemm_p3_planes_stats(A_img, W_img, M, N, K, stats_out, w_scale=1.0, bias=None, R1=None, relu=False, ln_stats=None, ln_tiles=0,
+                         ln_colsum=None, tile_rows=0):
+    lib = _lib()
+    ah, al, ra = A_img
+    wh, wl, rw = W_img
+    Mp = round_up(M, 128)
+    lib.pfhip_op_plane_image_bytes.restype = ctypes.c_size_t
+    lib.pfhip_op_plane_image_bytes.argtypes = [_ci, _ci]
+    nb = int(lib.pfhip_op_plane_image_bytes(Mp, N))
+    P = (torch.zeros(nb, dtype=torch.uint8, device=ah.device), torch.zeros(nb, dtype=torch.uint8, device=ah.device), Mp)
+    lib.pfhip_op_gemm_p3_planes_stats.argtypes = [_vp, _vp, _ci, _vp, _vp, _ci, ctypes.c_float, _vp, _vp, _ci, _vp, _vp, _ci, _ci, _ci, _ci,
+                                                  _ci, _vp, _ci, _vp, _vp, _ci, _vp]
+    _ck(lib.pfhip_op_gemm_p3_planes_stats(_p(ah), _p(al), ra, _p(wh), _p(wl), rw, float(w_scale), _p(P[0]), _p(P[1]), Mp, _p(bias), _p(R1),
+                                          R1.stride(0) if R1 is not None else 0, M, N, K, 1 if relu else 0, _p(ln_stats), ln_tiles,
+                                          _p(ln_colsum), _p(stats_out), tile_rows, _stream()), "gemm_p3_planes_stats")
+    return P
+
+
 def gemm_p3_wide_launches():
     lib = _lib()
     lib.pfhip_op_gemm_p3_wide_launches.restype = ctypes.c_long
diff --git a/include/pfhip_ops.h b/include/pfhip_ops.h
--- a/include/pfhip_ops.h
+++ b/include/pfhip_ops.h
@@ -24,6 +24,9 @@
 int pfhip_op_gemm_p3(const void* Ah, const void* Al, int rows_a, const void* Wh, const void* Wl, int rows_w, float w_scale, float* C, int ldc,
                      void* Ph, void* Pl, int rows_p, const float* bias, const float* R1, int ldr1, int M, int N, int K, int relu,
                      const float* ln_stats, int ln_tiles, const float* ln_colsum, float* stats_out, int tile_rows, void* stream);
+int pfhip_op_gemm_p3_planes_stats(const void* Ah, const void* Al, int rows_a, const void* Wh, const void* Wl, int rows_w, float w_scale, void* Ph,
+                                  void* Pl, int rows_p, const float* bias, const float* R1, int ldr1, int M, int N, int K, int relu,
+                                  const float* ln_stats, int ln_tiles, const float* ln_colsum, float* stats_out, int tile_rows, void* stream);
 int pfhip_op_gemm_p3_cols(const void* Ah, const void* Al, int rows_a, const void* Wh, const void* Wl, int rows_w, float w_scale, float* C, int ldc,
                           void* Ph, void* Pl, int rows_p, const float* bias, const float* R1, int ldr1, int M, int N, int K, int relu,
                           const float* ln_stats, int ln_tiles, const float* ln_colsum, float* stats_out, int tile_rows, int tile_cols,
@@ -33,6 +36,8 @@
                        int Dout, float eps, void* stream);
 int pfhip_op_fsmn(const float* v, int ldv, const float* w, const float* res, int ldres, float* out, int ldo,
                   const int* off, const int* len, int B, int max_len, int C, void* stream);
+int pfhip_op_dec_rowchain(const float* td, const float* g2, const float* b2, const float* w, float* xd, const float* g3, const float* b3,
+                          float* yd, const int* off, const int* len, int B, int max_len, int D, float eps, void* stream);
 int pfhip_op_fsmn_shift(const float* v, int ldv, const float* w, const float* res, int ldres, float* out, int ldo,
                         const int* off, const int* len, int B, int max_len, int C, int shift, void* stream);
 int pfhip_op_attention(const float* Q, int ldq, const float* K, int ldk, const float* V, int ldv, float* O, int ldo,
```

Measured after the change: 40850 (median of 6 runs). About the same (+0.6%).
